# sohmandal/classpose

Hardware: AMD Instinct MI355X
Metric: wsi_tiles_per_sec (higher is better)
Workload: dtype bf16; 1 GPU; configs[1]: synthetic 10000x10000 WSI (1936 tiles), tile 256 / overlap 32, conic 7 classes, ViT-L ClassTransformer depth 24 random-init, batch 32 sub-tiles = 8 WSI tiles/step, every step a distinct batch of the rank's shard (tiles sharded k % n_gpus, at most 256 distinct batches resident, longer runs wrap) streamed pinned host -> hipMemcpyAsync inside the timed region (the reader decodes ahead int; slide=10000, tile=256, overlap=32, batch_subtiles=32, distinct_batches=142, records_gathered=2048, decode_ahead_batches_at_t0=4, device_resident_batches_at_t0=1

## Files before the change

classpose_amd/_lib.py:

```python
from __future__ import annotations

import ctypes as C
import os
import subprocess

_HERE = os.path.dirname(os.path.abspath(__file__))
LIB_PATH = os.path.join(_HERE, "libclasspose_hip.so")
DEBUG_LIB_PATH = os.path.join(_HERE, "libclasspose_hip_debug.so")
CSRC = os.path.join(_HERE, "csrc")

ABI_VERSION = 3
DT_BF16, DT_F16, DT_F32 = 0, 1, 2
DTYPE_CODE = {"bf16": DT_BF16, "fp16": DT_F16, "fp32": DT_F32}
PROF_KINDS = ("fc1", "attention", "qkv", "proj", "fc2", "patch_embed", "neck_head")
FC1_KERNEL_NAME = "k_gemm4w<GELU + folded LayerNorm, one wave per SIMD> = void k_gemm4w<1, 0, false>(Gemm4wArgs)"


class CpxTiling(C.Structure):
    _fields_ = [("H", C.c_int), ("W", C.c_int), ("ypad1", C.c_int), ("xpad1", C.c_int),
                ("Ly", C.c_int), ("Lx", C.c_int), ("ny", C.c_int), ("nx", C.c_int),
                ("bsize", C.c_int), ("augment", C.c_int),
                ("ystart", C.c_int * 16), ("xstart", C.c_int * 16)]


class CpxBlockWeights(C.Structure):
    _fields_ = [(n, C.c_void_p) for n in (
        "ln1_w", "ln1_b", "qkv_w", "qkv_b", "proj_w", "proj_b", "rel_h", "rel_w",
        "ln2_w", "ln2_b", "fc1_w", "fc1_b", "fc2_w", "fc2_b", "qkv_colsum", "fc1_colsum")]


class CpxConvOp(C.Structure):
    _fields_ = [("kind", C.c_int), ("src_a", C.c_int), ("src_b", C.c_int), ("dst", C.c_int),
                ("cin_a", C.c_int), ("cin_b", C.c_int), ("cout", C.c_int), ("h", C.c_int), ("w", C.c_int),
                ("relu", C.c_int), ("weight", C.c_void_p), ("bias", C.c_void_p)]


class CpxQcOp(C.Structure):
    _fields_ = [("kind", C.c_int), ("k", C.c_int), ("stride", C.c_int), ("pad", C.c_int), ("act", C.c_int),
                ("h_in", C.c_int), ("w_in", C.c_int), ("h_out", C.c_int), ("w_out", C.c_int),
                ("src_a", C.c_size_t), ("src_b", C.c_size_t), ("gate", C.c_size_t), ("res", C.c_size_t),
                ("dst", C.c_size_t),
                ("c_a", C.c_int), ("ld_a", C.c_int), ("up_a", C.c_int), ("c_b", C.c_int), ("ld_b", C.c_int),
                ("ld_res", C.c_int), ("c_out", C.c_int), ("ld_dst", C.c_int), ("c_red", C.c_int),
                ("w", C.c_void_p), ("bias", C.c_void_p), ("w2", C.c_void_p), ("bias2", C.c_void_p)]


class CpxNetWeights(C.Structure):
    _fields_ = [("depth", C.c_int), ("ncls", C.c_int), ("n_head_cols", C.c_int),
                ("ld_head", C.c_int), ("dtype", C.c_int), ("fuse_ln", C.c_int),
                ("pe_w", C.c_void_p), ("pe_b", C.c_void_p), ("pos", C.c_void_p),
                ("blocks", C.POINTER(CpxBlockWeights)),
                ("neck0_w", C.c_void_p), ("neck_ln1_w", C.c_void_p), ("neck_ln1_b", C.c_void_p),
                ("neck2_w", C.c_void_p), ("neck_ln2_w", C.c_void_p), ("neck_ln2_b", C.c_void_p),
                ("head_w", C.c_void_p), ("head_b", C.c_void_p),
                ("n_unet_ops", C.c_int), ("unet_ops", C.POINTER(CpxConvOp)), ("prof", C.c_void_p)]


class CpxWeightJob(C.Structure):
    _fields_ = [("op", C.c_int), ("dtype", C.c_int), ("n", C.c_longlong), ("K", C.c_int), ("reserved", C.c_int),
                ("src_host", C.c_void_p * 4), ("stage_off", C.c_size_t * 4), ("dst", C.c_void_p * 3)]


WJ_ROUND_HALF, WJ_ROUND_F32, WJ_COPY_F32, WJ_FOLD_LN = 0, 1, 2, 3


class CpxRecord(C.Structure):
    _fields_ = [("tile", C.c_int32), ("label", C.c_int32), ("cls", C.c_int32), ("area", C.c_int32),
                ("y0", C.c_int32), ("x0", C.c_int32), ("y1", C.c_int32), ("x1", C.c_int32),
                ("sum_y", C.c_int64), ("sum_x", C.c_int64)]


class CpxPqPair(C.Structure):
    _fields_ = [(n, C.c_int32) for n in ("image", "cls", "first_true", "first_pred", "inter", "area_true", "area_pred", "reserved")]


class CpxPqInst(C.Structure):
    _fields_ = [(n, C.c_int32) for n in ("image", "side", "cls", "first", "area", "reserved")]


class CpxCell(C.Structure):
    _fields_ = [("area", C.c_double), ("perimeter", C.c_double), ("cx", C.c_double), ("cy", C.c_double),
                ("n_pts", C.c_int32), ("offset", C.c_int32), ("valid", C.c_int32), ("cls", C.c_int32)]


_p, _i, _f, _d, _sz = C.c_void_p, C.c_int, C.c_float, C.c_double, C.c_size_t

SIGNATURES = {
    "cpx_abi_version": (_i, []),
    "cpx_last_error": (C.c_char_p, []),
    "cpx_build_id": (C.c_char_p, []),
    "cpx_normalize_stats_u8": (_i, [_p, _i, _i, _i, _i, _f, _i, _f, _p, _p, _p]),
    "cpx_normalize_apply_u8": (_i, [_p, _p, _i, _i, _i, _p, _p]),
    "cpx_resize_linear_u8": (_i, [_p, _i, _i, _i, _p, _i, _i, _p]),
    "cpx_make_subtiles": (_i, [_p, _p, _i, C.POINTER(CpxTiling), _p, _p]),
    "cpx_make_patches": (_i, [_p, _p, _i, C.POINTER(CpxTiling), _i, _p, _p]),
    "cpx_make_subtiles_f32": (_i, [_p, _p, _i, C.POINTER(CpxTiling), _p, _p]),
    "cpx_blend_subtiles": (_i, [_p, _i, _i, _i, C.POINTER(CpxTiling), _p, _p, _p, _p, _p]),
    "cpx_blend_subtiles_nchw": (_i, [_p, _p, _i, _i, C.POINTER(CpxTiling), _p, _p, _p, _p, _p]),
    "cpx_qc_forward": (_i, [C.POINTER(CpxQcOp), _i, _p, _i, _i, _i, _sz, _sz, _i, _i, _p, _p, _p, _sz, _p]),
    "cpx_round_weights": (_i, [_p, _p, C.c_longlong, _i, _i, _p]),
    "cpx_fold_layernorm": (_i, [_p, _p, _p, _p, _i, _i, _i, _p, _p, _p, _p]),
    "cpx_weights_build": (_i, [C.POINTER(CpxWeightJob), _i, _p, _sz, _p]),
    "cpx_net_workspace_bytes": (_sz, [_i, _i]),
    "cpx_net_forward": (_i, [C.POINTER(CpxNetWeights), _p, _i, _p, _p, _sz, _p]),
    "cpx_unet_workspace_bytes": (_sz, [C.POINTER(CpxConvOp), _i, _i, _i]),
    "cpx_unet_head_forward": (_i, [C.POINTER(CpxConvOp), _i, _p, _i, _p, _i, _i, _i, _p, _sz, _p]),
    "cpx_net_mlp_parts": (_i, [_i, _i]),
    "cpx_prof_create": (_i, [_i, _i, C.c_uint, C.POINTER(C.c_void_p)]),
    "cpx_prof_collect": (_i, [_p, C.POINTER(C.c_double), C.POINTER(C.c_int)]),
    "cpx_prof_collect_launches": (_i, [_p, C.POINTER(C.c_float), C.POINTER(C.c_int), _i, C.POINTER(C.c_int)]),
    "cpx_prof_destroy": (None, [_p]),
    "cpx_gemm": (_i, [_i, _p, _p, _i, _i, _i, _i, _p, _p, _p, _i, _p]),
    "cpx_gemm_uses_big_tile": (_i, [_i, _i, _i, _i]),
    "cpx_layernorm": (_i, [_i, _p, _p, _p, _i, _i, _f, _p, _p]),
    "cpx_attention": (_i, [_i, _p, _p, _p, _i, _p, _p, _p]),
    "cpx_gemm_bf16": (_i, [_p, _p, _i, _i, _i, _i, _p, _p, _p, _i, _p]),
    "cpx_conv3x3": (_i, [_i, _p, _p, _i, _i, _i, _i, _p, _p, _i, _p]),
    "cpx_gemm_ln": (_i, [_p, _p, _i, _i, _i, _i, _p, _p, _p, _i, _p, _p, _p, _p]),
    "cpx_row_stats": (_i, [_p, _i, _p, _p]),
    "cpx_layernorm_bf16": (_i, [_p, _p, _p, _i, _i, _f, _p, _p]),
    "cpx_attention_relpos": (_i, [_p, _p, _p, _i, _p, _p, _p]),
    "cpx_postproc_workspace_bytes": (_sz, [_i, _i, _i]),
    "cpx_postproc_max_labels": (_i, [_i, _i]),
    "cpx_postproc_launch_count": (C.c_ulonglong, []),
    "cpx_follow_flows": (_i, [_p, _p, _i, _i, _i, _f, _i, _p, _p, _p, _p]),
    "cpx_get_masks": (_i, [_p, _i, _i, _i, _d, _p, _p, _p, _p]),
    "cpx_remove_bad_flow_masks": (_i, [_p, _p, _i, _i, _i, _d, _p, _p, _p]),
    "cpx_fill_holes_and_remove_small_masks": (_i, [_p, _i, _i, _i, _i, _p, _p, _p]),
    "cpx_compute_class_masks": (_i, [_p, _p, _i, _i, _i, _i, _p, _p, _p]),
    "cpx_remove_border_instances": (_i, [_p, _p, _i, _i, _i, _p, _p]),
    "cpx_compute_masks": (_i, [_p, _p, _p, _i, _i, _i, _i, _f, _d, _i, _i, _d, _p, _p, _p, _p, _p]),
    "cpx_instance_records": (_i, [_p, _p, _i, _i, _i, _i, _p, _p, _p, _p]),
    "cpx_compute_masks_records": (_i, [_p, _p, _p, _i, _i, _i, _i, _f, _d, _i, _i, _d, _p, _p, _p, _i, _p, _p, _p, _p]),
    "cpx_resize_linear_f32": (_i, [_p, _i, _i, _i, _p, _i, _i, _p]),
    "cpx_resize_nearest": (_i, [_p, _i, _i, _i, _i, _p, _i, _i, _p]),
    "cpx_pq_workspace_bytes": (_sz, [_i, _i, _i, _i, _i]),
    "cpx_pq_stats": (_i, [_p, _p, _i, _p, _p, _i, _i, _i, _i, _d, _i, _i, _i, _p, _p, _p, _p, _p, _p, _p, _i, _p, _i, _p, _p, _sz, _p]),
    "cpx_net_neck_offset": (_sz, [_i, _i]),
    "cpx_patchify_f32": (_i, [_p, _i, _i, _i, _i, _p, _p]),
    "cpx_class_loss_workspace_bytes": (_sz, [_i, _i, _i, _i]),
    "cpx_class_loss": (_i, [_p, _i, _i, _p, _i, _i, _i, _i, _p, _f, _f, _f, _f, _f, _p, _p, _p, _p, _p, _p, _p, _p, _p, _sz, _p]),
    "cpx_head_wgrad_slab_rows": (_i, []),
    "cpx_head_wgrad_workspace_bytes": (_sz, [_i, _i]),
    "cpx_head_wgrad": (_i, [_p, _p, _i, _i, _i, _p, _p, _p, _sz, _p]),
    "cpx_adamw_step": (_i, [_p, _p, _p, _p, C.c_longlong, _d, _d, _d, _d, _d, _d, _d, _p]),
    "cpx_unet_wgrad_slab_rows": (_i, []),
    "cpx_unet_param_layout": (C.c_longlong, [C.POINTER(CpxConvOp), _i, C.POINTER(C.c_longlong), C.POINTER(C.c_longlong),
                                             C.POINTER(_i), C.POINTER(_i)]),
    "cpx_unet_refresh_operands": (_i, [C.POINTER(CpxConvOp), _i, _p, _i, _p]),
    "cpx_unet_backward_workspace_bytes": (_sz, [C.POINTER(CpxConvOp), _i, _i, _i]),
    "cpx_unet_grad_layout": (_i, [C.POINTER(CpxConvOp), _i, _i, _i, C.POINTER(_sz), C.POINTER(_i)]),
    "cpx_unet_head_backward": (_i, [C.POINTER(CpxConvOp), _i, _p, _i, _i, _p, _sz, _p, _p, _p, _sz, _p]),
    "cpx_net_backbone_offset": (_sz, [_i, _i]),
    "cpx_neck_train_workspace_bytes": (_sz, [_i, _i]),
    "cpx_neck_train_layout": (_i, [_i, _i, C.POINTER(_sz)]),
    "cpx_neck_forward_train": (_i, [C.POINTER(CpxNetWeights), _p, _i, _p, _p, _sz, _p]),
    "cpx_layernorm_backward_workspace_bytes": (_sz, [_i, _i]),
    "cpx_layernorm_backward": (_i, [_i, _p, _p, _p, _i, _i, _f, _p, _p, _p, _p, _sz, _p]),
    "cpx_blocks_train_workspace_bytes": (_sz, [_i, _i, _i]),
    "cpx_blocks_train_layout": (_i, [_i, _i, _i, C.POINTER(_sz)]),
    "cpx_blocks_forward_train": (_i, [C.POINTER(CpxNetWeights), _p, _i, _i, _p, _p, _sz, _p]),
    "cpx_block_grad_layout": (C.c_longlong, [C.POINTER(C.c_longlong)]),
    "cpx_blocks_backward_workspace_bytes": (_sz, [_i, _i]),
    "cpx_blocks_backward_slab_crops": (_i, []),
    "cpx_blocks_backward": (_i, [C.POINTER(CpxNetWeights), _p, _i, _i, _p, _sz, _p, _p, _p, _p, _sz, _p]),
    "cpx_blocks_backward_workspace_bytes_ex": (_sz, [_i, _i, _i]),
    "cpx_blocks_backward_ex": (_i, [C.POINTER(CpxNetWeights), _p, _i, _i, _p, _sz, _p, _i, _p, _p, _p, _sz, _p]),
    "cpx_gemm_tn_bf16": (_i, [_p, _p, _i, _i, _i, _i, _p, _i, _p]),
    "cpx_colsum_workspace_bytes": (_sz, [_i, _i]),
    "cpx_colsum_add": (_i, [_p, _i, _i, _p, _p, _sz, _p]),
    "cpx_layernorm_backward_bytes": (_sz, [_i, _i]),
    "cpx_attention_backward_workspace_bytes": (_sz, [_i]),
    "cpx_attention_backward": (_i, [_i, _p, _p, _p, _p, _p, _i, _p, _p, _p, _p, _sz, _p]),
    "cpx_attention_backward_bf16_workspace_bytes": (_sz, [_i]),
    "cpx_attention_backward_bf16": (_i, [_p, _p, _p, _p, _i, _p, _p, _p, _p, _sz, _p]),
    "cpx_blocks_backward_workspace_bytes_mp": (_sz, [_i, _i, _i, _i]),
    "cpx_blocks_backward_mp": (_i, [C.POINTER(CpxNetWeights), _p, _i, _i, _p, _sz, _p, _i, _i, _p, _p, _p, _sz, _p]),
    "cpx_blocks_backward_in": (_i, [C.POINTER(CpxNetWeights), _p, _i, _i, _p, _sz, _p, _i, _i, _p, _p, _p, _p, _sz, _p]),
    "cpx_gather_crops": (_i, [_i, _p, _i, C.POINTER(_i), _i, _p, _p, _p]),
    "cpx_scatter_crops": (_i, [_i, _p, _i, C.POINTER(_i), _i, _p, _p]),
    "cpx_blocks_train_workspace_bytes_drop": (_sz, [_i, _i, _i]),
    "cpx_blocks_forward_train_drop": (_i, [C.POINTER(CpxNetWeights), _p, _i, _i, _p, _p, _p, _sz, _p]),
    "cpx_blocks_backward_drop": (_i, [C.POINTER(CpxNetWeights), _p, _i, _i, _p, _p, _sz, _p, _i, _i, _p, _p, _p, _p, _sz, _p]),
    "cpx_embed_grad_layout": (C.c_longlong, [C.POINTER(C.c_longlong)]),
    "cpx_embed_backward_workspace_bytes": (_sz, [_i, _i, _i]),
    "cpx_embed_backward": (_i, [_i, _p, _p, _i, _i, _p, _p, _sz, _p]),
    "cpx_gelu_backward": (_i, [_p, _p, _sz, _p, _p]),
    "cpx_neck_grad_layout": (C.c_longlong, [C.POINTER(C.c_longlong)]),
    "cpx_neck_backward_workspace_bytes": (_sz, [_i, _i, _i, C.POINTER(_sz)]),
    "cpx_neck_backward": (_i, [C.POINTER(CpxNetWeights), _p, _i, _p, _sz, _p, _p, _p, _sz, _p]),
    "cpx_hed_jitter_u8": (_i, [_p, _i, _i, _i, _p, _p, _d, _d, _i, _p, _p, _p]),
    "cpx_warp_affine_u8": (_i, [_p, _p, _i, _i, _i, _p, _i, _i, _i, _p, _p, _p]),
    "cpx_warp_affine_f32": (_i, [_p, _p, _i, _i, _i, _p, _i, _i, _i, _p, _p, _p]),
    "cpx_normalize_stats_f32": (_i, [_p, _i, _i, _i, _i, _f, _i, _f, _p, _p]),
    "cpx_normalize_apply_f32": (_i, [_p, _p, _i, _i, _i, _p, _p]),
    "cpx_label_stats_workspace_bytes": (_sz, [_i, _i, _i, _i]),
    "cpx_label_stats": (_i, [_p, _p, _i, _i, _i, _i, _p, _p, _p, _p, _p, _p, _sz, _p]),
    "cpx_rasterize_workspace_bytes": (_sz, [C.c_longlong, C.c_longlong, _i, _i, _i]),
    "cpx_rasterize_polygons": (_i, [_p, _p, _p, _p, C.c_longlong, _i, _i, _i, _p, _p, _sz, _p]),
    "cpx_ids_to_classes": (_i, [_p, C.c_longlong, _p, _i, _p, _p]),
    "cpx_label_components_workspace_bytes": (_sz, [_i, _i, _i]),
    "cpx_label_components": (_i, [_p, _i, _i, _i, _i, _p, _p, _p, _sz, _p]),
    "cpx_distance_sq": (_i, [_p, _i, _i, _i, _p, _p, _sz, _p]),
    "cpx_split_workspace_bytes": (_sz, [_i, _i, _i, _i]),
    "cpx_split_touching": (_i, [_p, _i, _i, _i, _i, _i, _i, _i, _p, _p, _p, _p, _p, _p, _sz, _p]),
    "cpx_pool_byte_sums": (_i, [_p, _p, _p, _i, C.c_longlong, _p, _p, _p]),
    "cpx_warp_affine_pool_u8": (_i, [_p, _p, _p, _p, _i, C.c_longlong, _p, _p, _i, _p, _p, _p, _i, _i, _i, _i, _p, _p, _p, _p]),
    "cpx_stain_samples_workspace_bytes": (_sz, [_i, C.c_longlong]),
    "cpx_stain_samples": (_i, [_p, _p, _p, _i, C.c_longlong, _p, _d, _p, C.c_longlong, _p, _p, _p, _p, _sz, _p]),
    "cpx_he_stain_u8": (_i, [_p, _i, _i, _i, _p, _p, _p, _p, _p]),
    "cpx_warp_affine_pool_stain_u8": (_i, [_p, _p, _p, _p, _i, C.c_longlong, _p, _p, _i, _p, _p, _i, _p, _p, _p, _i, _i, _i, _p, _p,
                                           _p, _p]),
    "cpx_hbs_u8": (_i, [_p, _i, _i, _i, _p, _p, _p, _p, _p]),
    "cpx_blur_pool_rects_u8": (_i, [_p, _p, _p, _i, C.c_longlong, _p, _p, _p, _p, _p, _i, _i, _i, _p, _p, _i, _p, _p, _p, _p,
                                    C.c_longlong, _p, _p]),
    "cpx_warp_affine_pool_quality_u8": (_i, [_p, _p, _p, _p, _i, C.c_longlong, _p, _p, _i, _p, _p, _i, _p, _p, _p, _p, _p, _p, _p,
                                             C.c_longlong, _p, _p, _i, _i, _i, _p, _p, _p, _p]),
    "cpx_masks_to_flows": (_i, [_p, _i, _i, _i, _p, _p, _p, _p]),
    "cpx_warp_affine_pool_flow_f32": (_i, [_p, _p, _p, _i, C.c_longlong, _p, _p, _p, _i, _i, _i, _p, _p, _p]),
    "cpx_seg_loss_workspace_bytes": (_sz, [_i, _i, _i]),
    "cpx_seg_loss": (_i, [_p, _i, _p, _i, _i, _i, _f, _p, _p, _p, _p, _sz, _p]),
    "cpx_find_contours_ccomp_host": (_i, [_p, _i, _i, _p, _i, _p, _p, _p, _i]),
    "cpx_polygonize_workspace_bytes": (_sz, [_i, _i, _i, _i]),
    "cpx_polygonize_device": (_i, [_p, _p, _p, _i, _i, _i, _i, _d, _p, _p, _i, _p, _p, _p, _p]),
    "cpx_polygonize_host": (_i, [_p, _i, _i, _p, _i, _d, _d, _d, _p, _i, _p]),
    "cpx_dedup_pairs_workspace_bytes": (_sz, [_i, _i, _i]),
    "cpx_dedup_pairs": (_i, [_p, _i, _d, _d, _d, _i, _i, _d, _p, C.c_longlong, _p, _p, _sz, _p]),
    "cpx_write_geojson": (_i, [C.c_char_p, C.c_char_p, _p, C.c_int64, _p, _p, _p, _p, C.c_int64, _p, _i, _d, _d, _i]),
    "cpx_write_geojson_ex": (_i, [C.c_char_p, C.c_char_p, _p, C.c_int64, _p, _p, _p, _p, C.c_int64, _p, _i, _d, _d, _i, _p, _i, _p]),
    "cpx_instance_confidence_workspace_bytes": (_sz, [_i, _i, _i, _i, _i]),
    "cpx_instance_confidence": (_i, [_p, _p, _p, _p, _i, _i, _i, _i, _i, _p, _p, _p, _p, _sz, _p]),
}
_PRIVATE = {
    "cpx_gemm_set_variant": (None, [_i]),
    "cpx_attention_set_variant": (None, [_i]),
    "cpx_gemm_set_nt": (None, [_i]),
    "cpx_follow_set_early_exit": (None, [_i]),
    "cpx_blur_set_tile": (None, [_i]),
    "cpx_follow_set_lds_window": (None, [_i]),
    "cpx_gemm_set_reverse": (None, [_i]),
    "cpx_attention_set_xcd_order": (None, [_i]),
    "cpx_gemm_set_big": (None, [_i]),
    "cpx_gemm_set_persistent": (None, [_i]),
    "cpx_gemm_set_persistent_qkv": (None, [_i]),
    "cpx_postproc_set_fused": (None, [_i]),
    "cpx_gemm_set_direct": (None, [_i]),
    "cpx_gemm4w": (_i, [_p, _p, _i, _i, _i, _p, _p, _i, _p]),
    "cpx_gemm4w_set_variant": (None, [_i]),
    "cpx_gemm_set_4w": (None, [_i]),
    "cpx_net_set_mlp_parts": (None, [_i]),
    "cpx_gemm_set_balanced": (None, [_i]),
    "cpx_gemm_set_l2_block": (None, [_i]),
    "cpx_gemm_ln_dt": (_i, [_i, _p, _p, _i, _i, _i, _i, _p, _p, _p, _i, _p, _p, _p, _p]),
    "cpx_row_stats_dt": (_i, [_i, _p, _i, _p, _p]),
    "cpx_im2col3_f32_debug": (_i, [_p, _i, _p, _p]),
    "cpx_confidence_set_footprint": (None, [_i]),
    "cpx_unet_head_layout": (_i, [C.POINTER(CpxConvOp), _i, _i, _i, C.POINTER(_sz), C.POINTER(_i)]),
# ... 109 lines not shown
```

classpose_amd/csrc/cpx_gemm.hip:

```cpp
#include "cpx_internal.h"
#include <type_traits>

typedef __attribute__((ext_vector_type(8))) __bf16 bf16x8;
typedef __attribute__((ext_vector_type(8))) _Float16 f16x8;
typedef __attribute__((ext_vector_type(4))) float f32x4;

#define BM 128
#define BN 128
#define BK 64
#define GEMM_THREADS 256
#define TILE_BYTES (128 * 128)
#define STAGE_BYTES (2 * TILE_BYTES)

template <bool NT_POSSIBLE, bool WT_POSSIBLE = false>
__device__ __forceinline__ void st16(void *p, uint4 v, bool nt, bool wt = false) {
    if (WT_POSSIBLE && wt) {
        typedef unsigned u32x4_t __attribute__((ext_vector_type(4)));
        u32x4_t w = {v.x, v.y, v.z, v.w};
        if (NT_POSSIBLE && nt) asm volatile("global_store_dwordx4 %0, %1, off sc1 nt" ::"v"(p), "v"(w) : "memory");
        else asm volatile("global_store_dwordx4 %0, %1, off sc1" ::"v"(p), "v"(w) : "memory");
    } else if (NT_POSSIBLE && nt) {
        typedef unsigned u32x4_t __attribute__((ext_vector_type(4)));
        u32x4_t w = {v.x, v.y, v.z, v.w};
        __builtin_nontemporal_store(w, reinterpret_cast<u32x4_t *>(p));
    } else {
        *reinterpret_cast<uint4 *>(p) = v;
    }
}
struct GemmArgs {
    const unsigned short *A;
    const unsigned short *W;
    int M, N, K;
    const float *bias;
    const void *aux;
    void *out;
    int ld_out;
    int tiles_n, n_blocks;
    int l2_block;
    int rev_m;
    int nt_out;
    const float *ln_stats;
    const float *ln_colsum;
    float *stats_out;
    int conv_c;
};
#define LN_SLOTS 4
__device__ __forceinline__ float2 ln_mean_rstd(float4 a, float4 b, float inv_k) {
    const float sum = (a.x + a.z) + (b.x + b.z), sq = (a.y + a.w) + (b.y + b.w);
    const float mean = sum * inv_k;
    return make_float2(mean, rsqrtf(fmaxf(sq * inv_k - mean * mean, 0.f) + 1e-6f));
}
__device__ __forceinline__ void ln_row_params(const float *st, int m, float inv_k, float &mean, float &rstd) {
    const float4 a = *reinterpret_cast<const float4 *>(st + (size_t)m * 8);
    const float4 b = *reinterpret_cast<const float4 *>(st + (size_t)m * 8 + 4);
    const float2 p = ln_mean_rstd(a, b, inv_k);
    mean = p.x; rstd = p.y;
}
__device__ __forceinline__ float2 ln_row_scale(float4 a, float4 b, float inv_k) {
    const float2 p = ln_mean_rstd(a, b, inv_k);
    return make_float2(p.y, -p.x * p.y);
}

template <int CTRL, int ROW_MASK = 0xF>
__device__ __forceinline__ float dpp_add(float v) {
    return v + __int_as_float(__builtin_amdgcn_update_dpp(0, __float_as_int(v), CTRL, ROW_MASK, 0xF, false));
}
__device__ __forceinline__ float half_wave_sum(float v) {
    v = dpp_add<0xB1>(v);
    v = dpp_add<0x4E>(v);
    v = dpp_add<0x141>(v);
    v = dpp_add<0x140>(v);
    return dpp_add<0x142, 0xA>(v);
}

template <bool F16>
__device__ __forceinline__ f32x4 mfma16(const uint4 &a, const uint4 &b, f32x4 c) {
    if constexpr (F16)
        return __builtin_amdgcn_mfma_f32_16x16x32_f16(*reinterpret_cast<const f16x8 *>(&a),
                                                      *reinterpret_cast<const f16x8 *>(&b), c, 0, 0, 0);
    else
        return __builtin_amdgcn_mfma_f32_16x16x32_bf16(*reinterpret_cast<const bf16x8 *>(&a),
                                                       *reinterpret_cast<const bf16x8 *>(&b), c, 0, 0, 0);
}

__device__ __forceinline__ float gelu_erf(float x) {
    const float ax = fabsf(x);
    float p = -4.732933965e-04f;
    p = __fmaf_rn(p, ax, 7.084452800e-03f);
    p = __fmaf_rn(p, ax, -5.182713611e-02f);
    p = __fmaf_rn(p, ax, -4.599926953e-01f);
    p = __fmaf_rn(p, ax, -1.150787739e+00f);
    p = __fmaf_rn(p, ax, -1.000037638e+00f);
    const float q = __builtin_amdgcn_exp2f(p);
    return __fmaf_rn(-ax, q, fmaxf(x, 0.0f));
}

template <bool F16>
__device__ __forceinline__ unsigned short to_half(float f) {
    if constexpr (F16) { _Float16 h = (_Float16)f; return *reinterpret_cast<unsigned short *>(&h); }
    else return f32_to_bf16(f);
}
template <bool F16>
__device__ __forceinline__ unsigned pack2(float a, float b) {
    typedef __attribute__((ext_vector_type(2))) float f32x2_t;
    typedef __attribute__((ext_vector_type(2))) __bf16 bf16x2_t;
    typedef __attribute__((ext_vector_type(2))) _Float16 f16x2_t;
    const f32x2_t v = {a, b};
    if constexpr (F16) return __builtin_bit_cast(unsigned, __builtin_convertvector(v, f16x2_t));
    else return __builtin_bit_cast(unsigned, __builtin_convertvector(v, bf16x2_t));
}
template <bool F16>
__device__ __forceinline__ float from_half(unsigned short u) {
    if constexpr (F16) { return (float)*reinterpret_cast<_Float16 *>(&u); }
    else return bf16_to_f32(u);
}

__device__ uint4 g_zero_chunk;

template <bool GLDS, bool CONV = false>
__device__ __forceinline__ void stage_tile(const unsigned short *__restrict__ g, int ldk, int row0, int k0,
                                           char *lds, int tid, uint4 *regs, int conv_c = 0) {
    int dy = 0, dx = 0, c0 = 0;
    if constexpr (CONV) {
        const int tap = k0 / conv_c;
        c0 = k0 - tap * conv_c;
        dy = tap / 3 - 1; dx = tap - (tap / 3) * 3 - 1;
    }
#pragma unroll
    for (int q = 0; q < 4; ++q) {
        int L = q * GEMM_THREADS + tid;
        int row = L >> 3, pc = L & 7;
        int kc = pc ^ (row & 7);
        const unsigned short *src;
        if constexpr (CONV) {
            const int m = row0 + row, yy = ((m >> 5) & 31) + dy, xx = (m & 31) + dx;
            src = ((unsigned)yy < 32u && (unsigned)xx < 32u)
                      ? g + ((size_t)(m & ~1023) + yy * 32 + xx) * conv_c + c0 + kc * 8
                      : reinterpret_cast<const unsigned short *>(&g_zero_chunk);
        } else {
            src = g + (size_t)(row0 + row) * ldk + k0 + kc * 8;
        }
        if constexpr (GLDS) {
            char *base = lds + (q * GEMM_THREADS + (tid & ~63)) * 16;
            __builtin_amdgcn_global_load_lds((const __attribute__((address_space(1))) void *)src,
                                             (__attribute__((address_space(3))) void *)base, 16, 0, 0);
        } else {
            regs[q] = *reinterpret_cast<const uint4 *>(src);
        }
    }
}
__device__ __forceinline__ void write_tile(char *lds, int tid, const uint4 *regs) {
#pragma unroll
    for (int q = 0; q < 4; ++q) *reinterpret_cast<uint4 *>(lds + (q * GEMM_THREADS + tid) * 16) = regs[q];
}

template <int EPI, bool F16, bool GLDS, bool CONV = false>
__global__ void __launch_bounds__(GEMM_THREADS, 2) k_gemm(GemmArgs g) {
    extern __shared__ __attribute__((aligned(16))) char smem[];
    const int tid = threadIdx.x, lane = tid & 63, wave = tid >> 6;
    const int wm = wave >> 1, wn = wave & 1;
    const int bid = xcd_contiguous_id(blockIdx.x, g.n_blocks);
    const int tile_m = bid / g.tiles_n, tile_n = bid - tile_m * g.tiles_n;
    const int m0 = tile_m * BM, n0 = tile_n * BN;
    const int nk = g.K / BK;

    f32x4 acc[4][4];
#pragma unroll
    for (int i = 0; i < 4; ++i)
#pragma unroll
        for (int j = 0; j < 4; ++j) acc[i][j] = (f32x4){0.f, 0.f, 0.f, 0.f};

    uint4 ra[4], rw[4];
    stage_tile<GLDS, CONV>(g.A, g.K, m0, 0, smem, tid, ra, g.conv_c);
    stage_tile<GLDS>(g.W, g.K, n0, 0, smem + TILE_BYTES, tid, rw);
    if constexpr (!GLDS) { write_tile(smem, tid, ra); write_tile(smem + TILE_BYTES, tid, rw); }
    else asm volatile("s_waitcnt vmcnt(0)" ::: "memory");
    __syncthreads();

    const int fr = lane & 15, fq = lane >> 4;
    int offA[2], offW[2];
#pragma unroll
    for (int ks = 0; ks < 2; ++ks) {
        int pc = (ks * 4 + fq) ^ (fr & 7);
        offA[ks] = (wm * 64 + fr) * 128 + pc * 16;
        offW[ks] = TILE_BYTES + (wn * 64 + fr) * 128 + pc * 16;
    }
    for (int kt = 0; kt < nk; ++kt) {
        char *cur = smem + (kt & 1) * STAGE_BYTES;
        char *nxt = smem + ((kt + 1) & 1) * STAGE_BYTES;
        uint4 fa[2][4], fw[2][4];
#pragma unroll
        for (int ks = 0; ks < 2; ++ks)
#pragma unroll
            for (int i = 0; i < 4; ++i) {
                fa[ks][i] = *reinterpret_cast<const uint4 *>(cur + offA[ks] + i * 16 * 128);
                fw[ks][i] = *reinterpret_cast<const uint4 *>(cur + offW[ks] + i * 16 * 128);
            }
        __builtin_amdgcn_sched_barrier(0);
        if (kt + 1 < nk) {
            stage_tile<GLDS, CONV>(g.A, g.K, m0, (kt + 1) * BK, nxt, tid, ra, g.conv_c);
            stage_tile<GLDS>(g.W, g.K, n0, (kt + 1) * BK, nxt + TILE_BYTES, tid, rw);
        }
        __builtin_amdgcn_sched_barrier(0);
#pragma unroll
        for (int ks = 0; ks < 2; ++ks)
#pragma unroll
            for (int nb = 0; nb < 4; ++nb)
#pragma unroll
                for (int mb = 0; mb < 4; ++mb)
                    acc[nb][mb] = mfma16<F16>(fw[ks][nb], fa[ks][mb], acc[nb][mb]);
        __builtin_amdgcn_sched_barrier(0);
        if (kt + 1 < nk) {
            if constexpr (!GLDS) { write_tile(nxt, tid, ra); write_tile(nxt + TILE_BYTES, tid, rw); }
            else asm volatile("s_waitcnt vmcnt(0)" ::: "memory");
        }
        __syncthreads();
    }

#pragma unroll
    for (int mb = 0; mb < 4; ++mb) {
        const int m = m0 + wm * 64 + mb * 16 + fr;
#pragma unroll
        for (int nb = 0; nb < 4; ++nb) {
            const int n = n0 + wn * 64 + nb * 16 + fq * 4;
            f32x4 v = acc[nb][mb];
            if (g.ln_stats) {
                float mean, rstd;
                ln_row_params(g.ln_stats, m, 1.0f / g.K, mean, rstd);
                const float4 cs = *reinterpret_cast<const float4 *>(g.ln_colsum + n);
                v[0] = (v[0] - mean * cs.x) * rstd; v[1] = (v[1] - mean * cs.y) * rstd;
                v[2] = (v[2] - mean * cs.z) * rstd; v[3] = (v[3] - mean * cs.w) * rstd;
            }
            if (g.bias) {
                const float4 b = *reinterpret_cast<const float4 *>(g.bias + n);
                v[0] += b.x; v[1] += b.y; v[2] += b.z; v[3] += b.w;
            }
            if constexpr (EPI == CPX_EPI_GELU_BF16) {
#pragma unroll
                for (int r = 0; r < 4; ++r) v[r] = gelu_erf(v[r]);
            } else if constexpr (EPI == CPX_EPI_RELU_BF16) {
#pragma unroll
                for (int r = 0; r < 4; ++r) v[r] = fmaxf(v[r], 0.f);
            } else if constexpr (EPI == CPX_EPI_RESID_BF16) {
#pragma unroll
                for (int r = 0; r < 4; ++r) v[r] = from_half<F16>(to_half<F16>(v[r]));
                const uint2 rr = *reinterpret_cast<const uint2 *>((const unsigned short *)g.aux + (size_t)m * g.ld_out + n);
                v[0] += from_half<F16>(rr.x & 0xFFFF); v[1] += from_half<F16>(rr.x >> 16);
                v[2] += from_half<F16>(rr.y & 0xFFFF); v[3] += from_half<F16>(rr.y >> 16);
            } else if constexpr (EPI == CPX_EPI_POS_BF16) {
                const float4 p = *reinterpret_cast<const float4 *>((const float *)g.aux + (size_t)(m & 1023) * g.N + n);
                v[0] += p.x; v[1] += p.y; v[2] += p.z; v[3] += p.w;
            }
            if constexpr (EPI == CPX_EPI_F32) {
                *reinterpret_cast<float4 *>((float *)g.out + (size_t)m * g.ld_out + n) = make_float4(v[0], v[1], v[2], v[3]);
            } else if (EPI == CPX_EPI_QKV_BF16 && n >= 2048) {
                unsigned short *vT = (unsigned short *)g.aux;
                const size_t s_ = (size_t)(m >> 10), t_ = (size_t)(m & 1023);
#pragma unroll
                for (int r = 0; r < 4; ++r) {
                    const int c = n - 2048 + r;
                    vT[((s_ * 16 + (c >> 6)) * 64 + (c & 63)) * 1024 + t_] = to_half<F16>(v[r]);
                }
            } else {
                uint2 o;
                o.x = pack2<F16>(v[0], v[1]);
                o.y = pack2<F16>(v[2], v[3]);
                *reinterpret_cast<uint2 *>((unsigned short *)g.out + (size_t)m * g.ld_out + n) = o;
            }
        }
    }
}


typedef __attribute__((ext_vector_type(4))) unsigned u32x4;
#define G2_THREADS 512
#define G2_HALF 16384
#define G2_BUF 65536
#define G2_EPI_LD 528
#define G2_LN_OFF (256 * G2_EPI_LD)
#define G2_LDS_BYTES (G2_LN_OFF + 256 * 8)

template <int OFF>
__device__ __forceinline__ u32x4 lds_read128(unsigned addr) {
    u32x4 v;
    asm volatile("ds_read_b128 %0, %1 offset:%2" : "=v"(v) : "v"(addr), "n"(OFF));
    return v;
}
template <bool F16>
__device__ __forceinline__ f32x4 mfma16v(const u32x4 &a, const u32x4 &b, f32x4 c) {
    if constexpr (F16)
        return __builtin_amdgcn_mfma_f32_16x16x32_f16(__builtin_bit_cast(f16x8, a), __builtin_bit_cast(f16x8, b), c, 0, 0, 0);
    else
        return __builtin_amdgcn_mfma_f32_16x16x32_bf16(__builtin_bit_cast(bf16x8, a), __builtin_bit_cast(bf16x8, b), c, 0, 0, 0);
}
template <int HM>
__device__ __forceinline__ void g2_read_x(u32x4 (&fx)[4][2], unsigned b0, unsigned b1) {
    fx[0][0] = lds_read128<HM * G2_HALF + 0 * 2048>(b0); fx[0][1] = lds_read128<HM * G2_HALF + 0 * 2048>(b1);
    fx[1][0] = lds_read128<HM * G2_HALF + 1 * 2048>(b0); fx[1][1] = lds_read128<HM * G2_HALF + 1 * 2048>(b1);
    fx[2][0] = lds_read128<HM * G2_HALF + 2 * 2048>(b0); fx[2][1] = lds_read128<HM * G2_HALF + 2 * 2048>(b1);
    fx[3][0] = lds_read128<HM * G2_HALF + 3 * 2048>(b0); fx[3][1] = lds_read128<HM * G2_HALF + 3 * 2048>(b1);
}
template <int HN>
__device__ __forceinline__ void g2_read_w(u32x4 (&fw)[2][2], unsigned b0, unsigned b1) {
    fw[0][0] = lds_read128<(2 + HN) * G2_HALF + 0 * 2048>(b0); fw[0][1] = lds_read128<(2 + HN) * G2_HALF + 0 * 2048>(b1);
    fw[1][0] = lds_read128<(2 + HN) * G2_HALF + 1 * 2048>(b0); fw[1][1] = lds_read128<(2 + HN) * G2_HALF + 1 * 2048>(b1);
}
template <bool F16, bool FIRST = false>
__device__ __forceinline__ void g2_mma(f32x4 (&acc)[4][2], const u32x4 (&fx)[4][2], const u32x4 (&fw)[2][2]) {
    __builtin_amdgcn_s_setprio(1);
#pragma unroll
    for (int ks = 0; ks < 2; ++ks)
#pragma unroll
        for (int mb = 0; mb < 4; ++mb)
#pragma unroll
            for (int nb = 0; nb < 2; ++nb)
                acc[mb][nb] = mfma16v<F16>(fw[nb][ks], fx[mb][ks], (FIRST && ks == 0) ? (f32x4){0.f, 0.f, 0.f, 0.f} : acc[mb][nb]);
    __builtin_amdgcn_s_setprio(0);
}
#define G2_BAR() __builtin_amdgcn_s_barrier()
#define G2_LGKM0() do { asm volatile("s_waitcnt lgkmcnt(0)" ::: "memory"); __builtin_amdgcn_sched_barrier(0); } while (0)

#define G2_TILE_OF(bid, tiles_m, tile_m, tile_n)                                            \
    if (g.l2_block && ((tiles_m) & 7) == 0 && (g.tiles_n & 3) == 0) {                       \
        const int grp = bid >> 5, w_ = bid & 31, cgn = g.tiles_n >> 2, rgn = (tiles_m) >> 3; \
        const int rg = g.l2_block == 2 ? grp % rgn : grp / cgn, cg = g.l2_block == 2 ? grp / rgn : grp - rg * cgn; \
        tile_m = rg * 8 + (w_ >> 2);                                                        \
        tile_n = cg * 4 + (w_ & 3);                                                         \
    } else {                                                                                \
        tile_m = bid / g.tiles_n;                                                           \
        tile_n = bid - tile_m * g.tiles_n;                                                  \
    }
#define G2_FRAG_BASES(xb, wb)                                                               \
    _Pragma("unroll") for (int ks = 0; ks < 2; ++ks) {                                      \
        const unsigned sw = (unsigned)(((ks * 4 + fq) ^ (fr & 7)) << 4);                    \
        xb[0][ks] = lds0 + (wm * 64 + fr) * 128 + sw;                                       \
        wb[0][ks] = lds0 + (wn * 32 + fr) * 128 + sw;                                       \
        xb[1][ks] = xb[0][ks] + G2_BUF;                                                     \
        wb[1][ks] = wb[0][ks] + G2_BUF;                                                     \
    }
#define G2_PHASES(B, FIRST, C1, C2)                                                         \
                                                                                    \
        g2_read_w<0>(fw, wb[B][0], wb[B][1]);                                               \
        g2_read_x<0>(fx, xb[B][0], xb[B][1]);                                               \
        if (C1) stage(1, t_ + 1);                                                           \
        G2_BAR(); G2_LGKM0();                                                               \
        g2_mma<F16, FIRST>(acc[0][0], fx, fw);                                              \
        __builtin_amdgcn_sched_barrier(0); G2_BAR();                                        \
                                                                                    \
        g2_read_w<1>(fw, wb[B][0], wb[B][1]);                                               \
        if (C1) stage(2, t_ + 1);                                                           \
        G2_BAR(); G2_LGKM0();                                                               \
        g2_mma<F16, FIRST>(acc[0][1], fx, fw);                                              \
        __builtin_amdgcn_sched_barrier(0); G2_BAR();                                        \
                                                                                    \
        g2_read_x<1>(fx, xb[B][0], xb[B][1]);                                               \
        if (C2) stage(0, t_ + 2);                                                           \
        G2_BAR(); G2_LGKM0();                                                               \
        g2_mma<F16, FIRST>(acc[1][1], fx, fw);                                              \
        __builtin_amdgcn_sched_barrier(0); G2_BAR();                                        \
                                                                                    \
        g2_read_w<0>(fw, wb[B][0], wb[B][1]);                                               \
        if (C2) { stage(3, t_ + 2); asm volatile("s_waitcnt vmcnt(4)" ::: "memory"); }      \
        else if (C1) asm volatile("s_waitcnt vmcnt(0)" ::: "memory");                       \
        G2_BAR(); G2_LGKM0();                                                               \
        g2_mma<F16, FIRST>(acc[1][0], fx, fw);                                              \
        __builtin_amdgcn_sched_barrier(0); G2_BAR();
#define G2_EPI_VALUE(v, rs, nm, cs, b)                                                      \
    {                                                                                       \
        if constexpr (LN_IN) {                                                              \
            v[0] = fmaf(v[0], rs, fmaf(nm, (cs).x, (b).x)); v[1] = fmaf(v[1], rs, fmaf(nm, (cs).y, (b).y)); \
            v[2] = fmaf(v[2], rs, fmaf(nm, (cs).z, (b).z)); v[3] = fmaf(v[3], rs, fmaf(nm, (cs).w, (b).w)); \
        } else {                                                                            \
            v[0] += (b).x; v[1] += (b).y; v[2] += (b).z; v[3] += (b).w;                     \
        }                                                                                   \
        if constexpr (EPI == CPX_EPI_GELU_BF16) {                                           \
            _Pragma("unroll") for (int r = 0; r < 4; ++r) v[r] = gelu_erf(v[r]);            \
        } else if constexpr (EPI == CPX_EPI_RELU_BF16) {                                    \
            _Pragma("unroll") for (int r = 0; r < 4; ++r) v[r] = fmaxf(v[r], 0.f);          \
        }                                                                                   \
    }
#define G2_STAGE_VT(v, nl, ml)                                                              \
    {                                                                                       \
        const unsigned p01 = pack2<F16>(v[0], v[1]), p23 = pack2<F16>(v[2], v[3]);          \
        *reinterpret_cast<unsigned short *>(smem + (nl + 0) * G2_EPI_LD + ml * 2) = (unsigned short)p01; \
        *reinterpret_cast<unsigned short *>(smem + (nl + 1) * G2_EPI_LD + ml * 2) = (unsigned short)(p01 >> 16); \
        *reinterpret_cast<unsigned short *>(smem + (nl + 2) * G2_EPI_LD + ml * 2) = (unsigned short)p23; \
        *reinterpret_cast<unsigned short *>(smem + (nl + 3) * G2_EPI_LD + ml * 2) = (unsigned short)(p23 >> 16); \
    }
#define G2_STORE_VT_ROWS(STORE)                                                             \
    {                                                                                       \
        unsigned short *vT = (unsigned short *)g.aux;                                       \
        const size_t s_ = (size_t)(m0 >> 10), t0 = (size_t)(m0 & 1023);                     \
        _Pragma("unroll 4") for (int it = 0; it < 16; ++it) {                               \
            const int row = it * 16 + (tid >> 5);                                           \
            const int c = n0 - 2048 + row;                                                  \
            uint4 v_ = *reinterpret_cast<const uint4 *>(smem + row * G2_EPI_LD + c16 * 16); \
            unsigned short *p_ = vT + ((s_ * 16 + (c >> 6)) * 64 + (c & 63)) * 1024 + t0 + c16 * 8; \
            STORE;                                                                          \
        }                                                                                   \
    }
#define G2_ADD_RESID(v, rres_it)                                                            \
    {                                                                                       \
        const uint4 rr = rres_it;                                                           \
        unsigned a[4] = {v.x, v.y, v.z, v.w}, b[4] = {rr.x, rr.y, rr.z, rr.w};              \
        _Pragma("unroll") for (int i = 0; i < 4; ++i) {                                     \
            float lo = from_half<F16>(a[i] & 0xFFFF) + from_half<F16>(b[i] & 0xFFFF);       \
            float hi = from_half<F16>(a[i] >> 16) + from_half<F16>(b[i] >> 16);             \
// ... 374 lines not shown
            const unsigned ldb = (unsigned)g.ld_out * 2u;
            const unsigned ovoff = (unsigned)(wm * 64 + fr) * ldb + (unsigned)(wn * 32 + ((fq & 1) << 4) + ((fq >> 1) << 3)) * 2u;
            const unsigned so0 = (unsigned)m0 * ldb + (unsigned)n0 * 2u;
#pragma unroll
            for (int hm = 0; hm < 2; ++hm) {
                float ln_rs[4], ln_nm[4];
                if constexpr (LN_IN) {
#pragma unroll
                    for (int mb = 0; mb < 4; ++mb) {
                        const float2 pr = *reinterpret_cast<const float2 *>(smem + G2P_TAIL + (hm * 128 + wm * 64 + mb * 16 + fr) * 8);
                        ln_rs[mb] = pr.x; ln_nm[mb] = pr.y;
                    }
                }
#pragma unroll
                for (int hn = 0; hn < 2; ++hn) {
                    float4 b[2], cs[2];
#pragma unroll
                    for (int nb = 0; nb < 2; ++nb) {
                        const int nl = hn * 128 + wn * 32 + nb * 16 + fq * 4;
                        b[nb] = *reinterpret_cast<const float4 *>(smem + G2P_TAIL + 2048 + nl * 4);
                        cs[nb] = make_float4(0.f, 0.f, 0.f, 0.f);
                        if constexpr (LN_IN) cs[nb] = *reinterpret_cast<const float4 *>(smem + G2P_TAIL + 3072 + nl * 4);
                    }
#pragma unroll
                    for (int mb = 0; mb < 4; ++mb) {
                        unsigned pk[2][2];
#pragma unroll
                        for (int nb = 0; nb < 2; ++nb) {
                            f32x4 vv = acc[hm][hn][mb][nb];
                            G2_EPI_VALUE(vv, ln_rs[mb], ln_nm[mb], cs[nb], b[nb])
                            pk[nb][0] = pack2<F16>(vv[0], vv[1]);
                            pk[nb][1] = pack2<F16>(vv[2], vv[3]);
                        }
                        const auto r0 = __builtin_amdgcn_permlane16_swap(pk[0][0], pk[1][0], false, false);
                        const auto r1 = __builtin_amdgcn_permlane16_swap(pk[0][1], pk[1][1], false, false);
                        const u32x4 o = {r0[0], r1[0], r0[1], r1[1]};
                        __builtin_amdgcn_raw_buffer_store_b128(o, rsrcO, ovoff, so0 + (unsigned)(hm * 128 + mb * 16) * ldb + (unsigned)hn * 256u, 0);
                    }
                }
            }
            G2_BAR();
        } else {
            if constexpr (EPI != CPX_EPI_RESID_BF16) {
                if (has_next) prefetch_next();
            }
            char *stg = smem + G2P_STG_OFF;
#pragma unroll
            for (int hm = 0; hm < 2; ++hm) {
                uint4 rres[8];
                if constexpr (EPI == CPX_EPI_RESID_BF16) {
#pragma unroll
                    for (int it = 0; it < 8; ++it)
                        rres[it] = *reinterpret_cast<const uint4 *>((const unsigned short *)g.aux +
                                                                    (size_t)(m0 + hm * 128 + it * 16 + (tid >> 5)) * g.ld_out + n0 + c16 * 8);
                }
                float ln_rs[4], ln_nm[4];
                if constexpr (LN_IN) {
#pragma unroll
                    for (int mb = 0; mb < 4; ++mb) {
                        const float2 pr = *reinterpret_cast<const float2 *>(smem + G2P_TAIL + (hm * 128 + wm * 64 + mb * 16 + fr) * 8);
                        ln_rs[mb] = pr.x; ln_nm[mb] = pr.y;
                    }
                }
#pragma unroll
                for (int hn = 0; hn < 2; ++hn)
#pragma unroll
                    for (int nb = 0; nb < 2; ++nb) {
                        const int nl = hn * 128 + wn * 32 + nb * 16 + fq * 4;
                        const float4 b = *reinterpret_cast<const float4 *>(smem + G2P_TAIL + 2048 + nl * 4);
                        float4 cs = make_float4(0.f, 0.f, 0.f, 0.f);
                        if constexpr (LN_IN) cs = *reinterpret_cast<const float4 *>(smem + G2P_TAIL + 3072 + nl * 4);
#pragma unroll
                        for (int mb = 0; mb < 4; ++mb) {
                            const int mlh = wm * 64 + mb * 16 + fr;
                            f32x4 vv = acc[hm][hn][mb][nb];
                            G2_EPI_VALUE(vv, ln_rs[mb], ln_nm[mb], cs, b)
                            uint2 o;
                            o.x = pack2<F16>(vv[0], vv[1]);
                            o.y = pack2<F16>(vv[2], vv[3]);
                            *reinterpret_cast<uint2 *>(stg + mlh * G2_EPI_LD + nl * 2) = o;
                        }
                    }
                asm volatile("s_waitcnt lgkmcnt(0)" ::: "memory");
                G2_BAR();
#pragma unroll
                for (int it = 0; it < 8; ++it) {
                    const int mlh = it * 16 + (tid >> 5);
                    uint4 vv = *reinterpret_cast<const uint4 *>(stg + mlh * G2_EPI_LD + c16 * 16);
                    const int ml = hm * 128 + mlh;
                    const size_t go = (size_t)(m0 + ml) * g.ld_out + n0 + c16 * 8;
                    if constexpr (EPI == CPX_EPI_RESID_BF16) G2_ADD_RESID(vv, rres[it])
                    st16<EPI == CPX_EPI_QKV_BF16, EPI == CPX_EPI_RESID_BF16 || EPI == CPX_EPI_QKV_BF16>((unsigned short *)g.out + go, vv, (g.nt_out & (n0 < 1024 ? 1 : 2)) != 0,
                                                                                        (g.nt_out & (EPI == CPX_EPI_QKV_BF16 ? 16 : 8)) != 0);
                    if constexpr (STATS) g2_row_stats<F16>(vv, c16, g.stats_out, (size_t)(m0 + ml), tile_n);
                }
                asm volatile("s_waitcnt lgkmcnt(0)" ::: "memory");
                G2_BAR();
            }
        }
        if (!has_next) break;
        prefetched = next_issued;
        v = vn; m0 = m0n; n0 = n0n; tile_n = tile_nn;
    }
}
#undef G2_TILE_OF
#undef G2_FRAG_BASES
#undef G2_PHASES
#undef G2_EPI_VALUE
#undef G2_STAGE_VT
#undef G2_STORE_VT_ROWS
#undef G2_ADD_RESID

CPX_SWITCH(g_gemm_persist, 1);
CPX_SWITCH(g_gemm_variant, 1);
CPX_SWITCH(g_gemm_l2, 1);
CPX_SWITCH(g_gemm_persist_qkv, 1);
CPX_SWITCH(g_gemm_rev, 0);
CPX_SWITCH(g_gemm_big, 1);
CPX_SWITCH(g_gemm_bal, 1);
CPX_SWITCH(g_gemm_direct, 1);
CPX_SWITCH(g_gemm_nt, 15);
CPX_SWITCH(g_gemm_4w, 1);
#ifdef CPX_DEBUG
extern "C" void cpx_gemm_set_persistent(int on) { g_gemm_persist = on; }
extern "C" void cpx_gemm_set_variant(int glds) { g_gemm_variant = glds; }
extern "C" void cpx_gemm_set_persistent_qkv(int on) { g_gemm_persist_qkv = on; }
extern "C" void cpx_gemm_set_l2_block(int on) { g_gemm_l2 = on; }
extern "C" void cpx_gemm_set_reverse(int on) { g_gemm_rev = on; }
extern "C" void cpx_gemm_set_big(int on) { g_gemm_big = on; }
extern "C" void cpx_gemm_set_direct(int on) { g_gemm_direct = on; }
extern "C" void cpx_gemm_set_balanced(int on) { g_gemm_bal = on; }
extern "C" void cpx_gemm_set_4w(int on) { g_gemm_4w = on; }
extern "C" void cpx_gemm_set_nt(int on) { g_gemm_nt = on; }
#endif

#define CPX_F16_DISPATCH(f16, F16, ...)                               \
    do {                                                              \
        if (f16) { constexpr bool F16 = true; __VA_ARGS__; }          \
        else { constexpr bool F16 = false; __VA_ARGS__; }             \
    } while (0)
template <auto KERNEL, int LDS_BYTES>
static void gemm_allow_lds() {
    static CpxOncePerDevice once;
    once([] { (void)hipFuncSetAttribute((const void *)KERNEL, hipFuncAttributeMaxDynamicSharedMemorySize, LDS_BYTES); });
}
static int gemm_cu_count() {
    int dev = 0, cus = 256;
    (void)hipGetDevice(&dev);
    (void)hipDeviceGetAttribute(&cus, hipDeviceAttributeMultiprocessorCount, dev);
    return cus > 0 ? cus : 256;
}

int cpx_gemm_half_uses_big_tile(int M, int N, int K, int epilogue) {
    if (epilogue == CPX_EPI_F32) return 0;
    if (!g_gemm_big || M % 256 || N % 256 || K < 128) return 0;
    if ((K / 64) % 2 && epilogue != CPX_EPI_POS_BF16) return 0;
    return (M / 256) * (N / 256) >= 256;
}

template <int EPI, bool F16, int FLAGS>
static void launch_gemm256_tiles(const GemmArgs &a, hipStream_t s) {
    gemm_allow_lds<k_gemm256<EPI, F16, FLAGS>, G2_LDS_BYTES>();
    hipLaunchKernelGGL((k_gemm256<EPI, F16, FLAGS>), dim3(a.n_blocks), dim3(G2_THREADS), G2_LDS_BYTES, s, a);
}
template <int EPI, bool F16, int FLAGS>
static void launch_gemm256_flags(const GemmArgs &a, hipStream_t s) {
    const bool qkv_balanced = EPI == CPX_EPI_QKV_BF16 && g_gemm_persist_qkv && (a.n_blocks / a.tiles_n) % 64 == 0 && a.tiles_n == 12;
    const bool fits32 = (size_t)a.M * (size_t)a.K * 2 < ((size_t)1 << 31) && (size_t)a.N * (size_t)a.K * 2 < ((size_t)1 << 31);
    if (g_gemm_persist && fits32 && (EPI != CPX_EPI_QKV_BF16 || qkv_balanced)) {
        gemm_allow_lds<k_gemm256p<EPI, F16, FLAGS>, G2P_LDS_BYTES>();
        static const int n_cu = gemm_cu_count();
        if (EPI == CPX_EPI_QKV_BF16) {
            if (n_cu == 256) {
                GemmArgs b = a;
                b.l2_block = 3;
                hipLaunchKernelGGL((k_gemm256p<EPI, F16, FLAGS>), dim3(256), dim3(G2_THREADS), G2P_LDS_BYTES, s, b);
                return;
            }
        } else {
            const int grid = a.n_blocks < n_cu ? a.n_blocks : n_cu;
            hipLaunchKernelGGL((k_gemm256p<EPI, F16, FLAGS>), dim3(grid), dim3(G2_THREADS), G2P_LDS_BYTES, s, a);
            return;
        }
    }
    launch_gemm256_tiles<EPI, F16, FLAGS>(a, s);
}

template <int EPI, bool F16>
static bool launch_gemm256(const GemmArgs &a0, hipStream_t s) {
    if constexpr (EPI == CPX_EPI_F32) return false;
    else {
        if (!cpx_gemm_half_uses_big_tile(a0.M, a0.N, a0.K, EPI)) return false;
        GemmArgs a = a0;
        a.tiles_n = a.N / 256; a.n_blocks = (a.M / 256) * (a.N / 256);
        constexpr bool PRODUCER = EPI == CPX_EPI_RESID_BF16 || EPI == CPX_EPI_POS_BF16;
        constexpr int F1 = PRODUCER ? G2F_STATS : G2F_LN;
        const bool f1 = PRODUCER ? a.stats_out != nullptr : a.ln_stats != nullptr;
        if constexpr (EPI == CPX_EPI_POS_BF16) {
            if (!f1) launch_gemm256_tiles<EPI, F16, 0>(a, s);
            else launch_gemm256_tiles<EPI, F16, G2F_STATS>(a, s);
            return true;
        } else {
            if constexpr (EPI == CPX_EPI_GELU_BF16) {
                if (g_gemm_4w && f1 && a.bias && a.K >= 256 && (a.K / 64) % 2 == 0 &&
                    cpx_gemm4w_gelu_ln(F16 ? 1 : 0, a.A, a.W, a.M, a.N, a.K, a.bias, a.ln_stats, a.ln_colsum, a.out, a.ld_out, s))
                    return true;
            }
            constexpr bool DIRECT_OK = EPI == CPX_EPI_GELU_BF16
#ifdef CPX_DEBUG
                                       || (EPI != CPX_EPI_RESID_BF16 && EPI != CPX_EPI_QKV_BF16)
#endif
                ;
            constexpr bool BAL_OK = EPI == CPX_EPI_RESID_BF16 && !F16;
            const bool bal = BAL_OK && g_gemm_bal != 0 && f1 && a.K >= 256;
            if constexpr (DIRECT_OK) {
                if ((EPI == CPX_EPI_GELU_BF16 ? g_gemm_direct != 0 : g_gemm_direct == 2) && (size_t)a.M * (size_t)a.ld_out * 2 < ((size_t)1 << 31)) {
                    if (f1) launch_gemm256_flags<EPI, F16, F1 | G2F_DIRECT>(a, s);
                    else launch_gemm256_flags<EPI, F16, G2F_DIRECT>(a, s);
                    return true;
                }
            }
            if constexpr (BAL_OK) {
                if (bal) {
                    launch_gemm256_flags<EPI, F16, F1 | G2F_BAL>(a, s);
                    return true;
                }
            }
            if (f1) launch_gemm256_flags<EPI, F16, F1>(a, s);
            else launch_gemm256_flags<EPI, F16, 0>(a, s);
            return true;
        }
    }
}

template <int EPI>
static void launch_gemm(const GemmArgs &a, hipStream_t s, bool f16) {
    bool big;
    CPX_F16_DISPATCH(f16, F16, big = launch_gemm256<EPI, F16>(a, s));
    if (big) return;
    dim3 grid(a.n_blocks), block(GEMM_THREADS);
    size_t lds = 2 * STAGE_BYTES;
#ifdef CPX_DEBUG
    if (!g_gemm_variant) {
        CPX_F16_DISPATCH(f16, F16, hipLaunchKernelGGL((k_gemm<EPI, F16, false>), grid, block, lds, s, a));
        return;
    }
#endif
    CPX_F16_DISPATCH(f16, F16, hipLaunchKernelGGL((k_gemm<EPI, F16, true>), grid, block, lds, s, a));
}

template <bool F16>
__device__ __forceinline__ void row_stats_emit(const uint4 a, const uint4 b, int lane, size_t row, float *__restrict__ st) {
    const unsigned u[8] = {a.x, a.y, a.z, a.w, b.x, b.y, b.z, b.w};
    float sm = 0.f, sq = 0.f;
#pragma unroll
    for (int i = 0; i < 8; ++i) {
        const float lo = from_half<F16>(u[i] & 0xFFFF), hi = from_half<F16>(u[i] >> 16);
        sm += lo + hi; sq += lo * lo + hi * hi;
    }
#pragma unroll
    for (int o = 32; o > 0; o >>= 1) { sm += __shfl_xor(sm, o); sq += __shfl_xor(sq, o); }
    if (lane < 4) *reinterpret_cast<float2 *>(st + (row * LN_SLOTS + lane) * 2) = lane == 0 ? make_float2(sm, sq) : make_float2(0.f, 0.f);
}
template <bool F16>
__global__ void __launch_bounds__(256) k_row_stats(const unsigned short *__restrict__ x, int rows,
                                                   float *__restrict__ st) {
    const int lane = threadIdx.x & 63, row = blockIdx.x * 4 + (threadIdx.x >> 6);
    if (row >= rows) return;
    const unsigned short *xr = x + (size_t)row * 1024 + lane * 16;
    const uint4 a = *reinterpret_cast<const uint4 *>(xr), b = *reinterpret_cast<const uint4 *>(xr + 8);
    row_stats_emit<F16>(a, b, lane, (size_t)row, st);
}

template <int NV, int STATS>
__global__ void __launch_bounds__(256) k_move_crop_rows(const uint4 *__restrict__ src, uint4 *__restrict__ dst, CpxCropList list, int scatter,
                                                        float *__restrict__ st) {
    const int lane = threadIdx.x & 63, tok = blockIdx.x * 4 + (threadIdx.x >> 6);
    const size_t crow = (size_t)(list.first + blockIdx.y) * 1024 + tok, frow = (size_t)list.crop[blockIdx.y] * 1024 + tok;
    const uint4 *s = src + (scatter ? crow : frow) * (64 * NV) + lane * NV;
    uint4 *d = dst + (scatter ? frow : crow) * (64 * NV) + lane * NV;
    uint4 v[NV];
#pragma unroll
    for (int i = 0; i < NV; ++i) v[i] = s[i];
#pragma unroll
    for (int i = 0; i < NV; ++i) d[i] = v[i];
    if constexpr (STATS != 0) row_stats_emit<STATS == 2>(v[0], v[1], lane, crow, st);
}
int cpx_move_crop_rows_run(int dtype, const void *src, void *dst, const CpxCropList &list, int scatter, float *stats, hipStream_t s) {
    const dim3 grid(256, list.n), block(256);
    const uint4 *a = (const uint4 *)src;
    uint4 *b = (uint4 *)dst;
    if (dtype == CPX_DT_F32) hipLaunchKernelGGL((k_move_crop_rows<4, 0>), grid, block, 0, s, a, b, list, scatter, stats);
    else if (!stats || scatter) hipLaunchKernelGGL((k_move_crop_rows<2, 0>), grid, block, 0, s, a, b, list, scatter, stats);
    else if (dtype == CPX_DT_F16) hipLaunchKernelGGL((k_move_crop_rows<2, 2>), grid, block, 0, s, a, b, list, scatter, stats);
    else hipLaunchKernelGGL((k_move_crop_rows<2, 1>), grid, block, 0, s, a, b, list, scatter, stats);
    CPX_CHECK_LAUNCH();
    return CPX_OK;
}
int cpx_row_stats_half(int dtype, const void *x, int rows, float *stats, void *stream) {
    CPX_REQUIRE(x && stats && rows > 0 && (dtype == CPX_DT_BF16 || dtype == CPX_DT_F16));
    CPX_F16_DISPATCH(dtype == CPX_DT_F16, F16,
                     hipLaunchKernelGGL(k_row_stats<F16>, dim3(cpx_cdiv(rows, 4)), dim3(256), 0, (hipStream_t)stream, (const unsigned short *)x, rows, stats));
    CPX_CHECK_LAUNCH();
    return CPX_OK;
}

extern "C" int cpx_row_stats(const void *x, int rows, float *stats, void *stream) {
    return cpx_row_stats_half(CPX_DT_BF16, x, rows, stats, stream);
}

static GemmArgs gemm_args(const void *A, const void *Wt, int M, int N, int K, const float *bias, const void *aux, void *out, int ld_out) {
    GemmArgs a = {};
    a.A = (const unsigned short *)A; a.W = (const unsigned short *)Wt;
    a.M = M; a.N = N; a.K = K; a.bias = bias; a.aux = aux; a.out = out; a.ld_out = ld_out;
    a.tiles_n = N / BN; a.n_blocks = (M / BM) * (N / BN);
    return a;
}

int cpx_gemm_half(int dtype, const void *A, const void *Wt, int M, int N, int K, int epilogue,
                  const float *bias, const void *aux, void *out, int ld_out,
                  const float *ln_stats, const float *ln_colsum, float *stats_out, void *stream) {
    CPX_REQUIRE(A && Wt && out && (dtype == CPX_DT_BF16 || dtype == CPX_DT_F16));
    const bool f16 = dtype == CPX_DT_F16;
    CPX_REQUIRE(M > 0 && N > 0 && K > 0 && M % BM == 0 && N % BN == 0 && K % BK == 0);
    CPX_REQUIRE(ld_out >= N && ld_out % 4 == 0);
    CPX_REQUIRE((epilogue != CPX_EPI_RESID_BF16 && epilogue != CPX_EPI_POS_BF16 && epilogue != CPX_EPI_QKV_BF16) || aux);
    CPX_REQUIRE(epilogue != CPX_EPI_QKV_BF16 || (N == 3072 && M % 1024 == 0));
    CPX_REQUIRE(!ln_stats || (ln_colsum && epilogue != CPX_EPI_RESID_BF16));
    CPX_REQUIRE(!stats_out || ((epilogue == CPX_EPI_RESID_BF16 || epilogue == CPX_EPI_POS_BF16) && N == 1024 && cpx_gemm_half_uses_big_tile(M, N, K, epilogue)));
    GemmArgs a = gemm_args(A, Wt, M, N, K, bias, aux, out, ld_out);
    a.ln_stats = ln_stats; a.ln_colsum = ln_colsum; a.stats_out = stats_out; a.l2_block = g_gemm_l2; a.nt_out = g_gemm_nt;
    a.rev_m = (g_gemm_rev && K >= 4096) ? 1 : 0;
    hipStream_t s = (hipStream_t)stream;
    switch (epilogue) {
        case CPX_EPI_BF16: launch_gemm<CPX_EPI_BF16>(a, s, f16); break;
        case CPX_EPI_GELU_BF16: launch_gemm<CPX_EPI_GELU_BF16>(a, s, f16); break;
        case CPX_EPI_RESID_BF16: launch_gemm<CPX_EPI_RESID_BF16>(a, s, f16); break;
        case CPX_EPI_F32: launch_gemm<CPX_EPI_F32>(a, s, f16); break;
        case CPX_EPI_POS_BF16: launch_gemm<CPX_EPI_POS_BF16>(a, s, f16); break;
        case CPX_EPI_RELU_BF16: launch_gemm<CPX_EPI_RELU_BF16>(a, s, f16); break;
        case CPX_EPI_QKV_BF16: launch_gemm<CPX_EPI_QKV_BF16>(a, s, f16); break;
        default: CPX_REQUIRE(!"unknown epilogue");
    }
    CPX_CHECK_LAUNCH();
    return CPX_OK;
}

int cpx_conv3_half(int dtype, const void *x, const void *Wt, int M, int N, int C, int epilogue, const float *bias,
                   void *out, int ld_out, void *stream) {
    CPX_REQUIRE(x && Wt && out && (dtype == CPX_DT_BF16 || dtype == CPX_DT_F16));
    CPX_REQUIRE(M > 0 && M % 1024 == 0 && N > 0 && N % BN == 0 && C > 0 && C % BK == 0);
    CPX_REQUIRE(ld_out >= N && ld_out % 4 == 0 && (epilogue == CPX_EPI_BF16 || epilogue == CPX_EPI_RELU_BF16));
    GemmArgs a = gemm_args(x, Wt, M, N, 9 * C, bias, nullptr, out, ld_out);
    a.conv_c = C;
    hipStream_t s = (hipStream_t)stream;
    dim3 grid(a.n_blocks), block(GEMM_THREADS);
    const size_t lds = 2 * STAGE_BYTES;
    const bool f16 = dtype == CPX_DT_F16;
    if (epilogue == CPX_EPI_BF16) CPX_F16_DISPATCH(f16, F16, hipLaunchKernelGGL((k_gemm<CPX_EPI_BF16, F16, true, true>), grid, block, lds, s, a));
    else CPX_F16_DISPATCH(f16, F16, hipLaunchKernelGGL((k_gemm<CPX_EPI_RELU_BF16, F16, true, true>), grid, block, lds, s, a));
    CPX_CHECK_LAUNCH();
    return CPX_OK;
}

extern "C" int cpx_conv3x3(int dtype, const void *x, const void *Wt, int M, int N, int C, int epilogue, const float *bias,
                           void *out, int ld_out, void *stream) {
    return cpx_conv3_half(dtype, x, Wt, M, N, C, epilogue, bias, out, ld_out, stream);
}

extern "C" int cpx_gemm_ln(const void *A, const void *Wt, int M, int N, int K, int epilogue,
                           const float *bias, const void *aux, void *out, int ld_out,
                           const float *ln_stats, const float *ln_colsum, float *stats_out, void *stream) {
    return cpx_gemm_half(CPX_DT_BF16, A, Wt, M, N, K, epilogue, bias, aux, out, ld_out, ln_stats, ln_colsum, stats_out, stream);
}
#ifdef CPX_DEBUG
extern "C" int cpx_gemm_ln_dt(int dtype, const void *A, const void *Wt, int M, int N, int K, int epilogue,
                              const float *bias, const void *aux, void *out, int ld_out,
                              const float *ln_stats, const float *ln_colsum, float *stats_out, void *stream) {
    return cpx_gemm_half(dtype, A, Wt, M, N, K, epilogue, bias, aux, out, ld_out, ln_stats, ln_colsum, stats_out, stream);
}
#endif
#ifdef CPX_DEBUG
extern "C" int cpx_row_stats_dt(int dtype, const void *x, int rows, float *stats, void *stream) {
    return cpx_row_stats_half(dtype, x, rows, stats, stream);
}
#endif
extern "C" int cpx_gemm_bf16(const void *A, const void *Wt, int M, int N, int K, int epilogue,
                             const float *bias, const void *aux, void *out, int ld_out, void *stream) {
    return cpx_gemm_half(CPX_DT_BF16, A, Wt, M, N, K, epilogue, bias, aux, out, ld_out, nullptr, nullptr, nullptr, stream);
}
extern "C" int cpx_gemm(int dtype, const void *A, const void *Wt, int M, int N, int K, int epilogue,
                        const float *bias, const void *aux, void *out, int ld_out, void *stream) {
    if (dtype == CPX_DT_F32)
        return cpx_gemm_f32((const float *)A, (const float *)Wt, M, N, K, epilogue, bias, (const float *)aux, (float *)out, ld_out, stream);
    return cpx_gemm_half(dtype, A, Wt, M, N, K, epilogue, bias, aux, out, ld_out, nullptr, nullptr, nullptr, stream);
}
extern "C" int cpx_gemm_uses_big_tile(int M, int N, int K, int epilogue) { return cpx_gemm_half_uses_big_tile(M, N, K, epilogue); }
```

classpose_amd/csrc/cpx_internal.h:

```cpp
#pragma once
#include "cpx_common.h"
#include <atomic>

struct CpxOncePerDevice {
    std::atomic<unsigned long long> done{0};
    template <class F>
    void operator()(F &&f) {
        int dev = 0;
        (void)hipGetDevice(&dev);
        const unsigned long long bit = 1ull << (dev & 63);
        if (!(done.load(std::memory_order_acquire) & bit)) {
            f();
            done.fetch_or(bit, std::memory_order_release);
        }
    }
};

enum { CPX_PROF_FC1 = 0, CPX_PROF_ATTN = 1, CPX_PROF_QKV = 2, CPX_PROF_PROJ = 3, CPX_PROF_FC2 = 4,
       CPX_PROF_PE = 5,
       CPX_PROF_TAIL = 6,
       CPX_PROF_KINDS = 7 };
struct CpxProf {
    hipEvent_t *ev = nullptr;
    int *kind = nullptr;
    int cap = 0, n = 0, stride = 1;
    int phase = 0;
    unsigned kinds_mask = 1;
};
static inline bool cpx_prof_begin(CpxProf *p, int kind, int layer, hipStream_t s) {
    if (!p || !p->ev || p->n >= p->cap || !((p->kinds_mask >> kind) & 1)) return false;
    if (kind < CPX_PROF_PE && ((layer + p->phase) % p->stride) != 0) return false;
    p->kind[p->n] = kind;
    return hipEventRecord(p->ev[2 * p->n], s) == hipSuccess;
}
static inline void cpx_prof_end(CpxProf *p, hipStream_t s) {
    (void)hipEventRecord(p->ev[2 * p->n + 1], s);
    ++p->n;
}

int cpx_gemm_half(int dtype, const void *A, const void *Wt, int M, int N, int K, int epilogue, const float *bias,
                  const void *aux, void *out, int ld_out, const float *ln_stats, const float *ln_colsum,
                  float *stats_out, void *stream);
int cpx_conv3_half(int dtype, const void *x, const void *Wt, int M, int N, int C, int epilogue, const float *bias,
                   void *out, int ld_out, void *stream);
int cpx_row_stats_half(int dtype, const void *x, int rows, float *stats, void *stream);
int cpx_gemm_half_uses_big_tile(int M, int N, int K, int epilogue);
#define CPX_CROP_LIST 64
struct CpxCropList { int n, first; int crop[CPX_CROP_LIST]; };
int cpx_move_crop_rows_run(int dtype, const void *src, void *dst, const CpxCropList &list, int scatter, float *stats, hipStream_t s);
int cpx_gemm4w_gelu_ln(int f16, const void *A, const void *W, int M, int N, int K, const float *bias, const float *ln_stats, const float *ln_colsum,
                       void *out, int ld_out, hipStream_t s);
int cpx_layernorm_half(int dtype, const void *x, const float *w, const float *b, int rows, int C, float eps,
                       void *out, void *stream);
int cpx_attention_half(int dtype, const void *qkv, const void *rel_h, const void *rel_w, int n_subtiles, void *vT_ws,
                       void *out, void *stream, bool transpose_v);
int cpx_attention2w_launch(int dtype, const void *qkv, const void *vT, const void *rel_h, const void *rel_w,
                           int n_subtiles, void *out, int xcd_order, hipStream_t s);

int cpx_gemm_f32(const float *A, const float *Wt, int M, int N, int K, int epilogue, const float *bias,
                 const float *aux, float *out, int ld_out, void *stream);
int cpx_layernorm_f32(const float *x, const float *w, const float *b, int rows, int C, float eps, float *out,
                      void *stream);
int cpx_attention_f32(const float *qkv, const float *rel_h, const float *rel_w, int n_subtiles, float *out,
                      void *stream);
int cpx_im2col3_f32(const float *x, int n_subtiles, float *out, void *stream);

__device__ __forceinline__ int xcd_contiguous_id(int v, int nblk) {
    const int nxcd = 8, q = nblk / nxcd, r = nblk % nxcd, x = v % nxcd;
    return (x < r ? x * (q + 1) : r * (q + 1) + (x - r) * q) + v / nxcd;
}

#define CPX_RUN(call) do { const int rc_ = (call); if (rc_) return rc_; } while (0)

struct NetWs { size_t off_x, off_xn, off_qkv, off_vt, off_ao, off_h, off_neck, off_neck2, off_st, off_col, total; };
NetWs cpx_net_ws(int nS, int dtype);
struct CpxBlockBufs { const void *x_in; void *x_mid, *x_out, *xn, *qkv, *vt, *ao, *hb; float *st; };
int cpx_net_block(const cpx_net_weights *w, int layer, int nS, const CpxBlockBufs &t, bool big_stats, CpxProf *prof, void *stream);
bool cpx_net_big_stats(const cpx_net_weights *w, int nS);
int cpx_net_tail(const cpx_net_weights *w, const void *x, int nS, void *y0, void *a1, void *y2, void *feat, void *col, float *head,
                 void *unet_ws, size_t unet_ws_bytes, void *stream);

int cpx_unet_head_run(int dtype, const cpx_conv_op *ops, int n_ops, const void *feat, int nS, float *head, int ld_head,
                      int col0, void *workspace, size_t ws_bytes, void *stream);
size_t cpx_unet_ws_bytes(int dtype, const cpx_conv_op *ops, int n_ops, int nS);
void cpx_unet_act_layout(int dtype, const cpx_conv_op *ops, int n_ops, int nS, size_t *off, int *ld);

static inline size_t es_of(int dtype) { return dtype == CPX_DT_F32 ? 4 : 2; }
static inline bool dtype_ok(int dtype) { return dtype == CPX_DT_BF16 || dtype == CPX_DT_F16 || dtype == CPX_DT_F32; }
static inline int up128(long long x) { return (int)((x + 127) / 128 * 128); }
static inline int up64(int x) { return (x + 63) / 64 * 64; }
struct OpDims { int taps, ctot, Npad, Kpad, Kp128, ho, wo, ld, rows_pad, rows_out_pad; size_t rows; };
static inline OpDims op_dims(const cpx_conv_op &o, int nS) {
    OpDims d;
    d.taps = o.kind == 0 ? 9 : (o.kind == 1 ? 4 : 1);
    d.ctot = o.cin_a + o.cin_b;
    d.Npad = up128(o.kind == 2 ? 4 * o.cout : o.cout);
    d.Kpad = up64(d.taps * d.ctot);
    d.Kp128 = up128(d.Kpad);
    d.ho = o.kind == 0 ? o.h : (o.kind == 1 ? o.h / 2 : o.h * 2);
    d.wo = o.kind == 0 ? o.w : (o.kind == 1 ? o.w / 2 : o.w * 2);
    d.rows = o.kind == 2 ? (size_t)nS * o.h * o.w : (size_t)nS * d.ho * d.wo;
    d.ld = up128(o.cout);
    d.rows_pad = up128((long long)d.rows);
    d.rows_out_pad = up128((long long)nS * d.ho * d.wo);
    return d;
}
struct CpxTensor { const char *p; int ld, c, h, w; };

#define CPX_DT_DISPATCH(dtype, DT, ...)                                                   \
    do {                                                                                  \
        if ((dtype) == CPX_DT_BF16) { constexpr int DT = CPX_DT_BF16; __VA_ARGS__; }      \
        else if ((dtype) == CPX_DT_F16) { constexpr int DT = CPX_DT_F16; __VA_ARGS__; }   \
        else { constexpr int DT = CPX_DT_F32; __VA_ARGS__; }                              \
    } while (0)
template <int DT>
__device__ __forceinline__ float load_f32(const void *p, size_t idx) {
    if constexpr (DT == CPX_DT_F32) return ((const float *)p)[idx];
    else if constexpr (DT == CPX_DT_F16) return (float)((const _Float16 *)p)[idx];
    else return bf16_to_f32(((const unsigned short *)p)[idx]);
}
template <int DT>
__device__ __forceinline__ float half_bits_to_f32(unsigned u) {
    if constexpr (DT == CPX_DT_F16) { const unsigned short h = (unsigned short)u; return (float)*reinterpret_cast<const _Float16 *>(&h); }
    else return bf16_to_f32((unsigned short)u);
}
template <int DT>
__device__ __forceinline__ float4 ld4(const void *p, size_t idx) {
    if constexpr (DT == CPX_DT_F32) return *reinterpret_cast<const float4 *>((const float *)p + idx);
    else {
        const uint2 a = *reinterpret_cast<const uint2 *>((const unsigned short *)p + idx);
        return make_float4(half_bits_to_f32<DT>(a.x & 0xFFFF), half_bits_to_f32<DT>(a.x >> 16), half_bits_to_f32<DT>(a.y & 0xFFFF),
                           half_bits_to_f32<DT>(a.y >> 16));
    }
}
typedef __attribute__((ext_vector_type(16))) float f32x16;
#define MFMA_F32(a, b, c) __builtin_amdgcn_mfma_f32_32x32x2f32((a), (b), (c), 0, 0, 0)
static inline dim3 grid1(size_t n) { return dim3((unsigned)((n + 255) / 256)); }
__device__ __forceinline__ double wave_sum(double x) {
#pragma unroll
    for (int o = 32; o > 0; o >>= 1) x += __shfl_xor(x, o, 64);
    return x;
}

struct AttnBwdLayout { size_t off_st[3], off_b[4], off_part, total; };
static inline AttnBwdLayout cpx_attn_bwd_layout(int nS) {
    AttnBwdLayout L; CpxArena a; const size_t n = (size_t)nS * 16 * 1024;
    for (int i = 0; i < 3; ++i) L.off_st[i] = a.take(n * sizeof(float));
    for (int i = 0; i < 4; ++i) L.off_b[i] = a.take(n * 32 * sizeof(float));
    L.off_part = a.take((size_t)nS * 4 * 2 * 4096 * sizeof(double));
    L.total = a.o;
    return L;
}
int cpx_attn_rel_grad_run(int dtype, const void *qkv, const float *Gh, const float *Gw, double *part, int nS, int add_rel, float *drel_h,
                          float *drel_w, void *stream);
int cpx_attention_backward_bf16_run(const void *qkv, const void *rel_h, const void *rel_w, const float *dO, int nS, float *dqkv, float *drel_h,
                                    float *drel_w, int add_rel, void *workspace, size_t workspace_bytes, void *stream);

#define UW_SLAB 512

struct UwArgs {
    const float *dy;
    const void *xa, *xb;
    int lda, ca, ldb, cb;
    int lh, lw;
    int rows, Npad, Kpad, k_valid;
    float *part_w; double *part_b;
};
struct DxArgs {
    const float *dcol; int ldc;
    int kind, ctot, coff, C;
    int lh, lw;
    size_t rows_src;
    float *gx; int ld_gx;
    const void *y; int ld_y; int mask;
};
size_t cpx_uwgrad_part_w_bytes(size_t rows, int Npad, int Kpad);
size_t cpx_uwgrad_workspace_bytes(size_t rows, int Npad, int Kpad);
int cpx_uwgrad_run(int dtype, int kind, const UwArgs &u, int n_valid, int bias_taps, int cout, float *dW, float *db, hipStream_t s);
int cpx_wt_run(int dtype, const void *w, int Npad, int Kpad, int Kp128, float *wt, hipStream_t s);
int cpx_dx_gather_run(int dtype, const DxArgs &g, hipStream_t s);
int cpx_transpose_f32_run(int dtype, const void *in, int R, int Cc, float *out, hipStream_t s);
```

classpose_amd/csrc/cpx_net.hip:

```cpp
#include "cpx_internal.h"
#include <algorithm>

typedef __attribute__((ext_vector_type(8))) __bf16 bf16x8;
typedef __attribute__((ext_vector_type(8))) _Float16 f16x8;

template <bool F16>
__device__ __forceinline__ f32x16 mfma32(const uint4 &a, const uint4 &b, f32x16 c) {
    if constexpr (F16)
        return __builtin_amdgcn_mfma_f32_32x32x16_f16(*reinterpret_cast<const f16x8 *>(&a),
                                                      *reinterpret_cast<const f16x8 *>(&b), c, 0, 0, 0);
    else
        return __builtin_amdgcn_mfma_f32_32x32x16_bf16(*reinterpret_cast<const bf16x8 *>(&a),
                                                       *reinterpret_cast<const bf16x8 *>(&b), c, 0, 0, 0);
}
template <bool F16>
__device__ __forceinline__ unsigned short h_from_f32(float f) {
    if constexpr (F16) { _Float16 h = (_Float16)f; return *reinterpret_cast<unsigned short *>(&h); }
    else return f32_to_bf16(f);
}
template <bool F16>
__device__ __forceinline__ float f32_from_h(unsigned short u) {
    if constexpr (F16) return (float)*reinterpret_cast<_Float16 *>(&u);
    else return bf16_to_f32(u);
}
// ... 291 lines not shown
    unsigned short *orow = out + (tok0 + qh * 32 + r) * 1024 + head * 64;
#pragma unroll
    for (int db = 0; db < 2; ++db)
#pragma unroll
        for (int g4 = 0; g4 < 4; g4 += 2) {
            const f32x16 &O = db ? O1 : O0;
            unsigned ax = pack2<F16>(O[4 * g4 + 0] * inv, O[4 * g4 + 1] * inv), ay = pack2<F16>(O[4 * g4 + 2] * inv, O[4 * g4 + 3] * inv);
            unsigned bx = pack2<F16>(O[4 * g4 + 4] * inv, O[4 * g4 + 5] * inv), by = pack2<F16>(O[4 * g4 + 6] * inv, O[4 * g4 + 7] * inv);
            const auto rx = __builtin_amdgcn_permlane32_swap(ax, bx, false, false);
            const auto ry = __builtin_amdgcn_permlane32_swap(ay, by, false, false);
            *reinterpret_cast<uint4 *>(orow + db * 32 + 8 * g4 + 8 * h2) = make_uint4(rx[0], ry[0], rx[1], ry[1]);
        }
}

CPX_SWITCH(g_att_xcd, 1);
CPX_SWITCH(g_att_v8, 2);
#ifdef CPX_DEBUG
extern "C" void cpx_attention_set_variant(int v8) { g_att_v8 = v8; }
extern "C" void cpx_attention_set_xcd_order(int v) { g_att_xcd = v; }
#endif
extern "C" int cpx_attention_relpos(const void *qkv, const void *rel_h, const void *rel_w,
                                    int n_subtiles, void *vT_ws, void *out, void *stream) {
    return cpx_attention_half(CPX_DT_BF16, qkv, rel_h, rel_w, n_subtiles, vT_ws, out, stream, true);
}
extern "C" int cpx_attention(int dtype, const void *qkv, const void *rel_h, const void *rel_w,
                             int n_subtiles, void *vT_ws, void *out, void *stream) {
    if (dtype == CPX_DT_F32)
        return cpx_attention_f32((const float *)qkv, (const float *)rel_h, (const float *)rel_w, n_subtiles, (float *)out, stream);
    return cpx_attention_half(dtype, qkv, rel_h, rel_w, n_subtiles, vT_ws, out, stream, true);
}
int cpx_attention_half(int dtype, const void *qkv, const void *rel_h, const void *rel_w, int n_subtiles,
                       void *vT_ws, void *out, void *stream, bool transpose_v) {
    CPX_REQUIRE(qkv && rel_h && rel_w && vT_ws && out && n_subtiles > 0);
    CPX_REQUIRE(dtype == CPX_DT_BF16 || dtype == CPX_DT_F16);
#ifdef CPX_DEBUG
    CPX_REQUIRE(g_att_v8 == 2 || g_att_v8 == 7);
#endif
    hipStream_t s = (hipStream_t)stream;
    if (transpose_v)
        hipLaunchKernelGGL(k_v_transpose, dim3(16, 16, n_subtiles), dim3(256), 0, s,
                           (const unsigned short *)qkv, (unsigned short *)vT_ws);
#ifdef CPX_DEBUG
    if (g_att_v8 == 7) {
        const dim3 grid4(8, 16, n_subtiles);
        static CpxOncePerDevice once4;
        once4([] {
            (void)hipFuncSetAttribute((const void *)k_attention4p<true>, hipFuncAttributeMaxDynamicSharedMemorySize, A4_LDS_BYTES);
            (void)hipFuncSetAttribute((const void *)k_attention4p<false>, hipFuncAttributeMaxDynamicSharedMemorySize, A4_LDS_BYTES);
        });
        if (dtype == CPX_DT_F16)
            hipLaunchKernelGGL((k_attention4p<true>), grid4, dim3(ATT_THREADS), A4_LDS_BYTES, s, (const unsigned short *)qkv, (const unsigned short *)vT_ws,
                               (const unsigned short *)rel_h, (const unsigned short *)rel_w, (unsigned short *)out, g_att_xcd);
        else
            hipLaunchKernelGGL((k_attention4p<false>), grid4, dim3(ATT_THREADS), A4_LDS_BYTES, s, (const unsigned short *)qkv, (const unsigned short *)vT_ws,
                               (const unsigned short *)rel_h, (const unsigned short *)rel_w, (unsigned short *)out, g_att_xcd);
        CPX_CHECK_LAUNCH();
        return CPX_OK;
    }
#endif
    return cpx_attention2w_launch(dtype, qkv, vT_ws, rel_h, rel_w, n_subtiles, out, g_att_xcd, s);
}

NetWs cpx_net_ws(int nS, int dtype) {
    NetWs w; CpxArena a; const size_t M = (size_t)nS * 1024, es = es_of(dtype);
    w.off_x = a.take(M * 1024 * es);
    w.off_xn = a.take(M * 1024 * es);
    w.off_qkv = a.take(M * 3072 * es);
    w.off_vt = a.take(es == 2 ? M * 1024 * es : 0);
    w.off_ao = a.take(M * 1024 * es);
    w.off_h = a.take(M * 4096 * es);
    w.off_neck = a.take(M * 256 * es);
    w.off_neck2 = a.take(M * 256 * es);
    w.off_st = a.take(es == 2 ? M * 8 * sizeof(float) : 0);
    w.off_col = a.take(es == 4 ? M * 2304 * es : 0);
    w.total = a.o;
    return w;
}
extern "C" size_t cpx_net_workspace_bytes(int n_subtiles, int dtype) {
    return n_subtiles > 0 ? cpx_net_ws(n_subtiles, dtype).total : 0;
}

extern "C" size_t cpx_net_neck_offset(int n_subtiles, int dtype) {
    if (n_subtiles <= 0 || dtype < CPX_DT_BF16 || dtype > CPX_DT_F32) return 0;
    return cpx_net_ws(n_subtiles, dtype).off_neck2;
}

extern "C" size_t cpx_net_backbone_offset(int n_subtiles, int dtype) {
    if (n_subtiles <= 0 || dtype < CPX_DT_BF16 || dtype > CPX_DT_F32) return (size_t)-1;
    return cpx_net_ws(n_subtiles, dtype).off_x;
}

extern "C" int cpx_prof_create(int max_launches, int stride, unsigned kinds_mask, void **out) {
    CPX_REQUIRE(out && max_launches > 0);
    CpxProf *p = new CpxProf();
    p->ev = new hipEvent_t[2 * (size_t)max_launches];
    p->kind = new int[max_launches];
    for (int i = 0; i < 2 * max_launches; ++i) {
        hipError_t e = hipEventCreate(&p->ev[i]);
        if (e != hipSuccess) {
            for (int j = 0; j < i; ++j) (void)hipEventDestroy(p->ev[j]);
            delete[] p->ev; delete[] p->kind; delete p;
            CPX_HIP(e);
        }
    }
    p->cap = max_launches; p->n = 0; p->stride = stride > 0 ? stride : 1;
    p->kinds_mask = kinds_mask ? kinds_mask : 1u;
    *out = p;
    return CPX_OK;
}
extern "C" int cpx_prof_collect(void *prof, double *ms_sum, int *count) {
    CpxProf *p = (CpxProf *)prof;
    CPX_REQUIRE(p && ms_sum && count);
    for (int k = 0; k < CPX_PROF_KINDS; ++k) { ms_sum[k] = 0.0; count[k] = 0; }
    for (int i = 0; i < p->n; ++i) {
        float ms = 0.f;
        CPX_HIP(hipEventElapsedTime(&ms, p->ev[2 * i], p->ev[2 * i + 1]));
        ms_sum[p->kind[i]] += ms;
        ++count[p->kind[i]];
    }
    p->n = 0;
    return CPX_OK;
}
extern "C" int cpx_prof_collect_launches(void *prof, float *ms, int *kind, int cap, int *n_out) {
    CpxProf *p = (CpxProf *)prof;
    CPX_REQUIRE(p && ms && kind && n_out && cap >= 0);
    for (int i = 0; i < p->n && i < cap; ++i) {
        CPX_HIP(hipEventElapsedTime(&ms[i], p->ev[2 * i], p->ev[2 * i + 1]));
        kind[i] = p->kind[i];
    }
    *n_out = p->n;
    return CPX_OK;
}
extern "C" void cpx_prof_destroy(void *prof) {
    CpxProf *p = (CpxProf *)prof;
    if (!p) return;
    for (int i = 0; i < 2 * p->cap; ++i) (void)hipEventDestroy(p->ev[i]);
    delete[] p->ev; delete[] p->kind; delete p;
}

CPX_SWITCH(g_mlp_parts, 1);
#ifdef CPX_DEBUG
extern "C" void cpx_net_set_mlp_parts(int on) { g_mlp_parts = on; }
#endif
extern "C" int cpx_net_mlp_parts(int n_subtiles, int dtype) {
    if (!g_mlp_parts || dtype == CPX_DT_F32 || n_subtiles < 32) return 1;
    return n_subtiles / 16;
}
static void mlp_part_rows(int n_subtiles, int parts, int pt, int &row0, int &rows) {
    row0 = pt * 16384;
    rows = pt + 1 < parts ? 16384 : n_subtiles * 1024 - row0;
}

int cpx_net_tail(const cpx_net_weights *w, const void *x, int nS, void *y0, void *a1, void *y2, void *feat, void *col, float *head,
                 void *unet_ws, size_t unet_ws_bytes, void *stream) {
    const int dt = w->dtype, M = nS * 1024;
    CPX_RUN(cpx_gemm(dt, x, w->neck0_w, M, 256, 1024, CPX_EPI_BF16, nullptr, nullptr, y0, 256, stream));
    CPX_RUN(cpx_layernorm(dt, y0, w->neck_ln1_w, w->neck_ln1_b, M, 256, 1e-6f, a1, stream));
    if (dt == CPX_DT_F32) {
        CPX_RUN(cpx_im2col3_f32((const float *)a1, nS, (float *)col, stream));
        CPX_RUN(cpx_gemm(dt, col, w->neck2_w, M, 256, 2304, CPX_EPI_BF16, nullptr, nullptr, y2, 256, stream));
    } else {
        CPX_RUN(cpx_conv3_half(dt, a1, w->neck2_w, M, 256, 256, CPX_EPI_BF16, nullptr, y2, 256, stream));
    }
    CPX_RUN(cpx_layernorm(dt, y2, w->neck_ln2_w, w->neck_ln2_b, M, 256, 1e-6f, feat, stream));
    CPX_RUN(cpx_gemm(dt, feat, w->head_w, M, w->ld_head, 256, CPX_EPI_F32, w->head_b, nullptr, head, w->ld_head, stream));
    if (w->n_unet_ops > 0) {
        const size_t need = cpx_unet_ws_bytes(dt, w->unet_ops, w->n_unet_ops, nS);
        CPX_REQUIRE(unet_ws_bytes >= need);
        CPX_RUN(cpx_unet_head_run(dt, w->unet_ops, w->n_unet_ops, feat, nS, head, w->ld_head, 192, unet_ws, need, stream));
    }
    return CPX_OK;
}

#define TIMED(kind_, layer_, call_) do { const bool t_ = cpx_prof_begin(prof, kind_, layer_, hs); CPX_RUN(call_); if (t_) cpx_prof_end(prof, hs); } while (0)

bool cpx_net_big_stats(const cpx_net_weights *w, int nS) {
    const int M = nS * 1024;
    return w->fuse_ln && w->dtype != CPX_DT_F32 && cpx_gemm_half_uses_big_tile(M, 1024, 1024, CPX_EPI_RESID_BF16) &&
           cpx_gemm_half_uses_big_tile(M, 1024, 4096, CPX_EPI_RESID_BF16);
}

int cpx_net_block(const cpx_net_weights *w, int layer, int nS, const CpxBlockBufs &t, bool big_stats, CpxProf *prof, void *stream) {
    const cpx_block_weights &b = w->blocks[layer];
    const int dt = w->dtype, M = nS * 1024;
    const bool f32 = dt == CPX_DT_F32;
    hipStream_t hs = (hipStream_t)stream;
    auto attention = [&] {
        return f32 ? cpx_attention_f32((const float *)t.qkv, (const float *)b.rel_h, (const float *)b.rel_w, nS, (float *)t.ao, stream)
                   : cpx_attention_half(dt, t.qkv, b.rel_h, b.rel_w, nS, t.vt, t.ao, stream, false);
    };
    if (w->fuse_ln) {
        TIMED(CPX_PROF_QKV, layer, cpx_gemm_half(dt, t.x_in, b.qkv_w, M, 3072, 1024, CPX_EPI_QKV_BF16, b.qkv_b, t.vt, t.qkv, 3072, t.st, b.qkv_colsum, nullptr, stream));
        TIMED(CPX_PROF_ATTN, layer, attention());
        TIMED(CPX_PROF_PROJ, layer, cpx_gemm_half(dt, t.ao, b.proj_w, M, 1024, 1024, CPX_EPI_RESID_BF16, b.proj_b, t.x_in, t.x_mid, 1024, nullptr, nullptr, big_stats ? t.st : nullptr, stream));
        if (!big_stats) CPX_RUN(cpx_row_stats_half(dt, t.x_mid, M, t.st, stream));
        const int parts = big_stats ? cpx_net_mlp_parts(nS, dt) : 1;
        for (int pt = 0; pt < parts; ++pt) {
            int r0, Mp;
            mlp_part_rows(nS, parts, pt, r0, Mp);
            const char *xp = (const char *)t.x_mid + (size_t)r0 * 1024 * 2;
            char *op = (char *)t.x_out + (size_t)r0 * 1024 * 2;
            float *stp = t.st + (size_t)r0 * 8;
            TIMED(CPX_PROF_FC1, layer, cpx_gemm_half(dt, xp, b.fc1_w, Mp, 4096, 1024, CPX_EPI_GELU_BF16, b.fc1_b, nullptr, t.hb, 4096, stp, b.fc1_colsum, nullptr, stream));
            TIMED(CPX_PROF_FC2, layer, cpx_gemm_half(dt, t.hb, b.fc2_w, Mp, 1024, 4096, CPX_EPI_RESID_BF16, b.fc2_b, xp, op, 1024, nullptr, nullptr, big_stats ? stp : nullptr, stream));
        }
        if (!big_stats) CPX_RUN(cpx_row_stats_half(dt, t.x_out, M, t.st, stream));
        return CPX_OK;
    }
    CPX_RUN(cpx_layernorm(dt, t.x_in, b.ln1_w, b.ln1_b, M, 1024, 1e-6f, t.xn, stream));
    TIMED(CPX_PROF_QKV, layer, cpx_gemm(dt, t.xn, b.qkv_w, M, 3072, 1024, f32 ? CPX_EPI_F32 : CPX_EPI_QKV_BF16, b.qkv_b, f32 ? nullptr : t.vt, t.qkv, 3072, stream));
    TIMED(CPX_PROF_ATTN, layer, attention());
    TIMED(CPX_PROF_PROJ, layer, cpx_gemm(dt, t.ao, b.proj_w, M, 1024, 1024, CPX_EPI_RESID_BF16, b.proj_b, t.x_in, t.x_mid, 1024, stream));
    CPX_RUN(cpx_layernorm(dt, t.x_mid, b.ln2_w, b.ln2_b, M, 1024, 1e-6f, t.xn, stream));
    TIMED(CPX_PROF_FC1, layer, cpx_gemm(dt, t.xn, b.fc1_w, M, 4096, 1024, CPX_EPI_GELU_BF16, b.fc1_b, nullptr, t.hb, 4096, stream));
    TIMED(CPX_PROF_FC2, layer, cpx_gemm(dt, t.hb, b.fc2_w, M, 1024, 4096, CPX_EPI_RESID_BF16, b.fc2_b, t.x_mid, t.x_out, 1024, stream));
    return CPX_OK;
}

extern "C" int cpx_net_forward(const cpx_net_weights *w, const void *patches, int nS, float *head,
                               void *workspace, size_t workspace_bytes, void *stream) {
    CPX_REQUIRE(w && patches && head && workspace && nS > 0);
    CPX_REQUIRE(w->depth > 0 && w->blocks && w->ld_head % 128 == 0 && w->ld_head >= w->n_head_cols);
    CPX_REQUIRE(dtype_ok(w->dtype) && (w->dtype != CPX_DT_F32 || !w->fuse_ln));
    const int dt = w->dtype, M = nS * 1024;
    const NetWs L = cpx_net_ws(nS, dt);
    CPX_REQUIRE(workspace_bytes >= L.total);
    char *ws = (char *)workspace;
    void *x = ws + L.off_x, *nk = ws + L.off_neck, *nk2 = ws + L.off_neck2;
    float *st = (float *)(ws + L.off_st);
    const CpxBlockBufs t = {x, x, x, ws + L.off_xn, ws + L.off_qkv, ws + L.off_vt, ws + L.off_ao, ws + L.off_h, st};
    CpxProf *prof = (CpxProf *)w->prof;
    if (prof) prof->phase = (prof->phase + 1) % prof->stride;
    hipStream_t hs = (hipStream_t)stream;
    const bool big_stats = cpx_net_big_stats(w, nS);
    const bool pe_stats = big_stats && cpx_gemm_half_uses_big_tile(M, 1024, 192, CPX_EPI_POS_BF16);
    TIMED(CPX_PROF_PE, 0, pe_stats ? cpx_gemm_half(dt, patches, w->pe_w, M, 1024, 192, CPX_EPI_POS_BF16, w->pe_b, w->pos, x, 1024, nullptr, nullptr, st, stream)
                                   : cpx_gemm(dt, patches, w->pe_w, M, 1024, 192, CPX_EPI_POS_BF16, w->pe_b, w->pos, x, 1024, stream));
    if (w->fuse_ln && !pe_stats) CPX_RUN(cpx_row_stats_half(dt, x, M, st, stream));
    for (int i = 0; i < w->depth; ++i) CPX_RUN(cpx_net_block(w, i, nS, t, big_stats, prof, stream));
    TIMED(CPX_PROF_TAIL, 0, cpx_net_tail(w, x, nS, nk, nk2, nk, nk2, ws + L.off_col, head, ws + L.total, workspace_bytes - L.total, stream));
    return CPX_OK;
}
#undef TIMED

template <int ES>
__global__ void __launch_bounds__(256) k_conv_gather(const char *__restrict__ a, int lda, int ca,
                                                     const char *__restrict__ b, int ldb, int cb,
                                                     int kind, int h, int w, size_t rows_out, int kpad,
                                                     char *__restrict__ out) {
    constexpr int EPC = 16 / ES;
    const int ctot = ca + cb, ccn = ctot / EPC, taps = kind == 0 ? 9 : (kind == 1 ? 4 : 1);
    const int chunks_per_row = kpad / EPC;
    size_t i = (size_t)blockIdx.x * 256 + threadIdx.x;
    if (i >= rows_out * chunks_per_row) return;
    size_t row = i / chunks_per_row;
    int ch = (int)(i - row * chunks_per_row);
    uint4 v = make_uint4(0, 0, 0, 0);
    const int ho = kind == 1 ? h >> 1 : h, wo = kind == 1 ? w >> 1 : w;
    if (ch < taps * ccn) {
        int tap = ch / ccn, cc = ch - tap * ccn;
        size_t s_ = row / (size_t)(ho * wo);
        int t = (int)(row - s_ * ho * wo), y = t / wo, x = t - y * wo;
        int yy, xx;
        if (kind == 0) { yy = y + tap / 3 - 1; xx = x + tap % 3 - 1; }
        else if (kind == 1) { yy = 2 * y + (tap >> 1); xx = 2 * x + (tap & 1); }
        else { yy = y; xx = x; }
        if ((unsigned)yy < (unsigned)h && (unsigned)xx < (unsigned)w) {
            size_t src_row = s_ * h * w + (size_t)yy * w + xx;
            int c = cc * EPC;
            v = c < ca ? *reinterpret_cast<const uint4 *>(a + (src_row * lda + c) * ES)
                       : *reinterpret_cast<const uint4 *>(b + (src_row * ldb + (c - ca)) * ES);
        }
    }
    *reinterpret_cast<uint4 *>(out + (row * kpad + (size_t)ch * EPC) * ES) = v;
}

template <int DT>
__global__ void __launch_bounds__(256) k_depth2space(const char *__restrict__ in, int ld_in, int cout,
                                                     int h, int w, size_t rows_in, char *__restrict__ out,
                                                     int ld_out, float *__restrict__ out_f32, int ld_f32, int col0) {
    constexpr int ES = DT == CPX_DT_F32 ? 4 : 2, EPC = 16 / ES;
    const int ccn = cout / EPC;
    size_t i = (size_t)blockIdx.x * 256 + threadIdx.x;
    if (i >= rows_in * 4 * ccn) return;
    size_t row = i / (4 * ccn);
    int rem = (int)(i - row * 4 * ccn), tap = rem / ccn, cc = rem - tap * ccn;
    size_t s_ = row / (size_t)(h * w);
    int t = (int)(row - s_ * h * w), y = t / w, x = t - y * w;
    size_t orow = s_ * 4 * h * w + (size_t)(2 * y + (tap >> 1)) * (2 * w) + 2 * x + (tap & 1);
    uint4 v = *reinterpret_cast<const uint4 *>(in + (row * ld_in + tap * cout + cc * EPC) * ES);
    if (out_f32) {
        float *o = out_f32 + orow * ld_f32 + col0 + cc * EPC;
        if constexpr (DT == CPX_DT_F32) {
            *reinterpret_cast<uint4 *>(o) = v;
        } else {
            const unsigned u[4] = {v.x, v.y, v.z, v.w};
#pragma unroll
            for (int k = 0; k < 4; ++k) { o[2 * k] = f32_from_h<DT == CPX_DT_F16>(u[k] & 0xFFFF); o[2 * k + 1] = f32_from_h<DT == CPX_DT_F16>(u[k] >> 16); }
        }
    } else {
        *reinterpret_cast<uint4 *>(out + (orow * ld_out + cc * EPC) * ES) = v;
    }
}

struct UnetLayout {
    size_t col_off, g_off, total;
    size_t off[64];
    int ld[64];
};
static void unet_layout(int dtype, const cpx_conv_op *ops, int n_ops, int nS, UnetLayout &L) {
    const size_t es = es_of(dtype);
    size_t col_max = 0, g_max = 0;
    for (int i = 0; i < n_ops; ++i) {
        const OpDims d = op_dims(ops[i], nS);
        col_max = std::max(col_max, (size_t)d.rows_pad * d.Kpad * es);
        if (ops[i].kind == 2) g_max = std::max(g_max, (size_t)d.rows_pad * d.Npad * es);
    }
    CpxArena a;
    L.col_off = a.take(col_max);
    L.g_off = a.take(g_max);
    for (int i = 0; i < n_ops && i < 64; ++i) {
        const OpDims d = op_dims(ops[i], nS);
        L.ld[i] = d.ld;
        L.off[i] = a.take((size_t)d.rows_out_pad * d.ld * es);
    }
    L.total = a.o + 1024;
}

size_t cpx_unet_ws_bytes(int dtype, const cpx_conv_op *ops, int n_ops, int nS) {
    if (!ops || n_ops <= 0 || n_ops > 64 || nS <= 0) return 0;
    UnetLayout L;
    unet_layout(dtype, ops, n_ops, nS, L);
    return L.total;
}
extern "C" size_t cpx_unet_workspace_bytes(const cpx_conv_op *ops, int n_ops, int nS, int dtype) {
    return cpx_unet_ws_bytes(dtype, ops, n_ops, nS);
}
void cpx_unet_act_layout(int dtype, const cpx_conv_op *ops, int n_ops, int nS, size_t *off, int *ld) {
    UnetLayout L;
    unet_layout(dtype, ops, n_ops, nS, L);
    for (int i = 0; i < n_ops && i < 64; ++i) { off[i] = L.off[i]; ld[i] = L.ld[i]; }
}
#ifdef CPX_DEBUG
extern "C" int cpx_unet_head_layout(const cpx_conv_op *ops, int n_ops, int nS, int dtype, size_t *dst_off, int *ld) {
    CPX_REQUIRE(ops && n_ops > 0 && n_ops <= 64 && nS > 0 && dst_off && ld && ops[n_ops - 1].kind == 2);
    UnetLayout L;
    unet_layout(dtype, ops, n_ops, nS, L);
    for (int i = 0; i < n_ops; ++i) { dst_off[i] = L.off[i]; ld[i] = L.ld[i]; }
    dst_off[n_ops - 1] = L.g_off;
    ld[n_ops - 1] = op_dims(ops[n_ops - 1], nS).Npad;
    return CPX_OK;
}
#endif

int cpx_unet_head_run(int dtype, const cpx_conv_op *ops, int n_ops, const void *feat, int nS, float *head,
                      int ld_head, int col0, void *workspace, size_t ws_bytes, void *stream) {
    CPX_REQUIRE(ops && n_ops > 0 && n_ops <= 64 && feat && head && workspace && nS > 0);
    CPX_REQUIRE(ws_bytes >= cpx_unet_ws_bytes(dtype, ops, n_ops, nS));
    hipStream_t s = (hipStream_t)stream;
    const size_t es = es_of(dtype);
    CpxTensor tens[66];
    tens[0] = {(const char *)feat, 256, 256, 32, 32};
    char *ws = (char *)workspace;
    UnetLayout lay;
    unet_layout(dtype, ops, n_ops, nS, lay);
    char *colbuf = ws + lay.col_off, *gbuf = ws + lay.g_off;
    const auto gather = es == 4 ? k_conv_gather<4> : k_conv_gather<2>;
    auto d2s = k_depth2space<CPX_DT_F32>;
    if (dtype != CPX_DT_F32) d2s = dtype == CPX_DT_F16 ? k_depth2space<CPX_DT_F16> : k_depth2space<CPX_DT_BF16>;
    for (int i = 0; i < n_ops; ++i) {
        const cpx_conv_op &o = ops[i];
        CPX_REQUIRE(o.dst > 0 && o.dst < 66 && o.src_a >= 0 && o.src_a < 66 && o.src_b < 66);
        CPX_REQUIRE(o.cin_a % 8 == 0 && o.cin_b % 8 == 0 && o.cout % 8 == 0 && o.weight && o.bias);
        const CpxTensor &A = tens[o.src_a];
        const CpxTensor Bz = {nullptr, 0, 0, 0, 0};
        const CpxTensor &B = o.src_b >= 0 ? tens[o.src_b] : Bz;
        CPX_REQUIRE(A.c == o.cin_a && A.h == o.h && A.w == o.w && (o.src_b < 0 || (B.c == o.cin_b && B.h == o.h && B.w == o.w)));
        if (o.kind == 2) CPX_REQUIRE(o.src_b < 0);
        const OpDims d = op_dims(o, nS);
        const bool convT = o.kind == 2;
        const dim3 grid_g((unsigned)((d.rows * (d.Kpad / (16 / es)) + 255) / 256));
        hipLaunchKernelGGL(gather, grid_g, dim3(256), 0, s, A.p, A.ld, o.cin_a, B.p, B.ld, convT ? 0 : o.cin_b, convT ? 3 : o.kind, o.h, o.w, d.rows, d.Kpad, colbuf);
        char *dst = ws + lay.off[i];
        const int rc = cpx_gemm(dtype, colbuf, o.weight, d.rows_pad, d.Npad, d.Kpad, !convT && o.relu ? CPX_EPI_RELU_BF16 : CPX_EPI_BF16, o.bias, nullptr,
                                convT ? gbuf : dst, d.Npad, stream);
        if (rc) return rc;
        if (convT) {
            const bool last = i == n_ops - 1;
            const dim3 grid((unsigned)((d.rows * 4 * (o.cout / (16 / es)) + 255) / 256));
            hipLaunchKernelGGL(d2s, grid, dim3(256), 0, s, gbuf, d.Npad, o.cout, o.h, o.w, d.rows, dst, d.ld, last ? head : nullptr, ld_head, col0);
        }
        tens[o.dst] = {dst, d.ld, o.cout, d.ho, d.wo};
    }
    CPX_CHECK_LAUNCH();
    return CPX_OK;
}
// ... 5 lines not shown
```

classpose_amd/csrc/cpx_pre.hip:

```cpp
#include "cpx_common.h"

#define NTHR 256

__device__ __forceinline__ void cv_linear_tap(int d, double scale, int slen, bool clamp_weight,
                                              int &s0, int &s1, int &w0, int &w1) {
    float f = (float)(((double)d + 0.5) * scale - 0.5);
    int s = (int)floorf(f);
    f -= (float)s;
    if (clamp_weight) {
        if (s < 0) { f = 0.f; s = 0; }
        if (s >= slen - 1) { f = 0.f; s = slen - 1; }
    }
    w0 = __float2int_rn((1.f - f) * 2048.f);
    w1 = __float2int_rn(f * 2048.f);
    s0 = min(max(s, 0), slen - 1);
    s1 = min(max(s + 1, 0), slen - 1);
}

__global__ void k_resize_linear_u8(const uint8_t *__restrict__ src, int sh, int sw,
                                   uint8_t *__restrict__ dst, int dh, int dw, double scale_x,
                                   double scale_y, int area2) {
    int p = blockIdx.x * NTHR + threadIdx.x;
    if (p >= dh * dw) return;
    int dy = p / dw, dx = p - dy * dw;
// ... 168 lines not shown
    return *reinterpret_cast<unsigned short *>(&h);
}
template <int DT>
__global__ void k_make_patches(const uint8_t *__restrict__ tiles, const float *__restrict__ stats,
                               TilingDev g, void *__restrict__ patches_v) {
    const int tok_per = (g.b / 8) * (g.b / 8);
    const int per_sub = tok_per * 24;
    int i = blockIdx.x * NTHR + threadIdx.x;
    if (i >= per_sub) return;
    int sub = blockIdx.y;
    int t = sub / (g.ny * g.nx), ji = sub - t * g.ny * g.nx;
    int j = ji / g.nx, ii_t = ji - j * g.nx;
    int tok = i / 24, r = i - tok * 24;
    int c = r >> 3, ii = r & 7;
    int ph = tok / (g.b / 8), pw = tok - ph * (g.b / 8);
    bool fy = g.augment && (ii_t & 1) && !(j & 1);
    bool fx = g.augment && (j & 1) && !(ii_t & 1);
    if (g.augment && (j & 1) && (ii_t & 1)) { fy = true; fx = true; }
    int y = 8 * ph + ii;
    int sy = fy ? g.b - 1 - y : y;
    union { unsigned short h[8]; uint4 v; } o;
    float f[8];
#pragma unroll
    for (int jj = 0; jj < 8; ++jj) {
        int x = 8 * pw + jj;
        int sx = fx ? g.b - 1 - x : x;
        float v = padded_px(tiles, stats, g, t, g.ys[j] + sy, g.xs[ii_t] + sx, c);
        f[jj] = v;
        o.h[jj] = DT == 1 ? f32_to_f16(v) : f32_to_bf16(v);
    }
    const size_t e = ((size_t)sub * tok_per + tok) * 192 + c * 64 + ii * 8;
    if constexpr (DT == 2) {
        float *patches = (float *)patches_v;
        *reinterpret_cast<float4 *>(patches + e) = make_float4(f[0], f[1], f[2], f[3]);
        *reinterpret_cast<float4 *>(patches + e + 4) = make_float4(f[4], f[5], f[6], f[7]);
    } else {
        *reinterpret_cast<uint4 *>((unsigned short *)patches_v + e) = o.v;
    }
}

__global__ void k_make_subtiles_f32(const uint8_t *__restrict__ tiles, const float *__restrict__ stats,
                                    TilingDev g, float *__restrict__ out) {
    int i = blockIdx.x * NTHR + threadIdx.x;
    int per = 3 * g.b * g.b;
    if (i >= per) return;
    int sub = blockIdx.y;
    int t = sub / (g.ny * g.nx), ji = sub - t * g.ny * g.nx;
    int j = ji / g.nx, ii_t = ji - j * g.nx;
    int c = i / (g.b * g.b), r = i - c * g.b * g.b;
    int y = r / g.b, x = r - y * g.b;
    bool fy = g.augment && (ii_t & 1) && !(j & 1);
    bool fx = g.augment && (j & 1) && !(ii_t & 1);
    if (g.augment && (j & 1) && (ii_t & 1)) { fy = true; fx = true; }
    int sy = fy ? g.b - 1 - y : y, sx = fx ? g.b - 1 - x : x;
    out[(size_t)sub * per + i] = padded_px(tiles, stats, g, t, g.ys[j] + sy, g.xs[ii_t] + sx, c);
}

extern "C" int cpx_make_patches(const uint8_t *tiles, const float *stats, int nT,
                                const cpx_tiling *tiling, int dtype, void *patches, void *stream) {
    TilingDev g; int rc = tiling_to_dev(tiling, &g); if (rc) return rc;
    CPX_REQUIRE(tiles && stats && patches && nT > 0 && dtype >= 0 && dtype <= 2);
    int per_sub = (g.b / 8) * (g.b / 8) * 24;
    const dim3 grid(cpx_cdiv(per_sub, NTHR), nT * g.ny * g.nx);
    if (dtype == 2) hipLaunchKernelGGL(k_make_patches<2>, grid, dim3(NTHR), 0, (hipStream_t)stream, tiles, stats, g, patches);
    else if (dtype == 1) hipLaunchKernelGGL(k_make_patches<1>, grid, dim3(NTHR), 0, (hipStream_t)stream, tiles, stats, g, patches);
    else hipLaunchKernelGGL(k_make_patches<0>, grid, dim3(NTHR), 0, (hipStream_t)stream, tiles, stats, g, patches);
    CPX_CHECK_LAUNCH();
    return CPX_OK;
}
extern "C" int cpx_make_subtiles(const uint8_t *tiles, const float *stats, int nT,
                                 const cpx_tiling *tiling, void *patches, void *stream) {
    return cpx_make_patches(tiles, stats, nT, tiling, 0, patches, stream);
}

extern "C" int cpx_make_subtiles_f32(const uint8_t *tiles, const float *stats, int nT,
                                     const cpx_tiling *tiling, float *subtiles, void *stream) {
    TilingDev g; int rc = tiling_to_dev(tiling, &g); if (rc) return rc;
    CPX_REQUIRE(tiles && stats && subtiles && nT > 0);
    hipLaunchKernelGGL(k_make_subtiles_f32, dim3(cpx_cdiv(3 * g.b * g.b, NTHR), nT * g.ny * g.nx),
                       dim3(NTHR), 0, (hipStream_t)stream, tiles, stats, g, subtiles);
    CPX_CHECK_LAUNCH();
    return CPX_OK;
}

template <bool TOKEN_MAJOR>
__global__ void k_blend(const float *__restrict__ src, const float *__restrict__ src2, int ld, int ncls,
                        TilingDev g, const double *__restrict__ taper, float *__restrict__ dP,
                        float *__restrict__ cellprob, float *__restrict__ logits) {
    int idx = blockIdx.x * NTHR + threadIdx.x;
    const int HW = g.H * g.W;
    if (idx >= HW) return;
    const int ch = blockIdx.z;
    size_t t = blockIdx.y;
    int Y = idx / g.W, X = idx - Y * g.W;
    int Yp = Y + g.ypad1, Xp = X + g.xpad1;
    const int tb = g.b / 8;
    float acc = 0.f;
    double navg = 0.0;
    for (int j = 0; j < g.ny; ++j) {
        int y = Yp - g.ys[j];
        if ((unsigned)y >= (unsigned)g.b) continue;
        for (int i = 0; i < g.nx; ++i) {
            int x = Xp - g.xs[i];
            if ((unsigned)x >= (unsigned)g.b) continue;
            bool fy = g.augment && (i & 1) && !(j & 1);
            bool fx = g.augment && (j & 1) && !(i & 1);
            if (g.augment && (j & 1) && (i & 1)) { fy = true; fx = true; }
            int sy = fy ? g.b - 1 - y : y, sx = fx ? g.b - 1 - x : x;
            size_t sub = (t * g.ny + j) * g.nx + i;
            float v;
            if (TOKEN_MAJOR) {
                int tok = (sy >> 3) * tb + (sx >> 3);
                int col = (ch < 3 ? ch * 64 : 192 + (ch - 3) * 64) + (sy & 7) * 8 + (sx & 7);
                v = src[(sub * tb * tb + tok) * (size_t)ld + col];
            } else {
                v = ch < 3 ? src[((sub * 3 + ch) * g.b + sy) * (size_t)g.b + sx]
                           : src2[((sub * ncls + (ch - 3)) * g.b + sy) * (size_t)g.b + sx];
            }
            if ((ch == 0 && fy) || (ch == 1 && fx)) v = -v;
            double m = taper[x] * taper[y];
            acc = (float)((double)acc + (double)v * m);
            navg = navg + m;
        }
    }
    float r = (float)((double)acc / navg);
    if (ch < 2) dP[(t * 2 + ch) * HW + idx] = r;
    else if (ch == 2) cellprob[t * HW + idx] = r;
    else logits[(t * ncls + (ch - 3)) * HW + idx] = r;
}

extern "C" int cpx_blend_subtiles(const float *head, int ld_head, int ncls, int nT,
                                  const cpx_tiling *tiling, const double *taper1d, float *dP,
                                  float *cellprob, float *logits, void *stream) {
    TilingDev g; int rc = tiling_to_dev(tiling, &g); if (rc) return rc;
    CPX_REQUIRE(head && taper1d && dP && cellprob && nT > 0 && ncls >= 0 && (ncls == 0 || logits));
    CPX_REQUIRE(ld_head >= 192 + ncls * 64);
    hipLaunchKernelGGL(k_blend<true>, dim3(cpx_cdiv(g.H * g.W, NTHR), nT, 3 + ncls), dim3(NTHR), 0,
                       (hipStream_t)stream, head, (const float *)nullptr, ld_head, ncls, g, taper1d,
                       dP, cellprob, logits);
    CPX_CHECK_LAUNCH();
    return CPX_OK;
}

extern "C" int cpx_blend_subtiles_nchw(const float *y, const float *y_class, int ncls, int nT,
                                       const cpx_tiling *tiling, const double *taper1d, float *dP,
                                       float *cellprob, float *logits, void *stream) {
    TilingDev g; int rc = tiling_to_dev(tiling, &g); if (rc) return rc;
    CPX_REQUIRE(y && taper1d && dP && cellprob && nT > 0 && ncls >= 0 && (ncls == 0 || (logits && y_class)));
    hipLaunchKernelGGL(k_blend<false>, dim3(cpx_cdiv(g.H * g.W, NTHR), nT, 3 + ncls), dim3(NTHR), 0,
                       (hipStream_t)stream, y, y_class, 0, ncls, g, taper1d, dP, cellprob, logits);
    CPX_CHECK_LAUNCH();
    return CPX_OK;
}
```

classpose_amd/engine.py:

```python
from __future__ import annotations

import os

import ctypes as C
import math
from dataclasses import dataclass

import numpy as np
import torch

from . import _lib
from ._lib import CpxBlockWeights, CpxConvOp, CpxNetWeights, CpxRecord, CpxTiling, check, ptr

PS = 8
BSIZE = 256
HALF_DTYPES = {"bf16": torch.bfloat16, "fp16": torch.float16}
NET_DTYPES = {**HALF_DTYPES, "fp32": torch.float32}


def make_tiling(H: int, W: int, bsize: int = BSIZE, augment: bool = False,
                tile_overlap: float = 0.1) -> CpxTiling:
    def pad(L):
        lpad = int(16 * math.ceil(L / 16) - L) if L >= bsize else bsize - L
        return 8 + lpad // 2, 8 + lpad - lpad // 2
# ... 194 lines not shown
        self.fts = fts
        if jobs:
            with torch.cuda.device(dev):
                stage = torch.empty(stage_bytes, dtype=torch.uint8, device=dev)
                arr = (_lib.CpxWeightJob * len(jobs))(*jobs)
                st = torch.cuda.current_stream(dev)
                check(L.cpx_weights_build(arr, len(jobs), stage.data_ptr(), stage_bytes, st.cuda_stream), "weights_build")
                st.synchronize()
                del stage
        sources.clear()
        return self

    def _build_unet_ops(self, sd, fts, out_ch, half, vec32):
        hd = {0: torch.bfloat16, 1: torch.float16, 2: torch.float32}[self.c.dtype]
        up = lambda x, m: (x + m - 1) // m * m
        p8 = lambda c: up(c, 8)
        ops = []

        def rounded(t):
            return t.detach().to(hd).float()

        def add(kind, src_a, src_b, cin_a, cin_b, cout, h, relu, wkey):
            w, b = rounded(sd[wkey + ".weight"]), rounded(sd[wkey + ".bias"])
            ca, cb, co = p8(cin_a), p8(cin_b), p8(cout)
            if kind == 2:
                wt = torch.zeros(2, 2, co, ca)
                wt[:, :, :cout, :cin_a] = w.permute(2, 3, 1, 0)
                wm = wt.reshape(4 * co, ca)
                bt = torch.zeros(4, co)
                bt[:, :cout] = b[None, :]
                bm = bt.reshape(-1)
            else:
                k = w.shape[-1]
                wt = torch.zeros(co, k, k, ca + cb)
                wk = w.permute(0, 2, 3, 1)
                wt[:cout, :, :, :cin_a] = wk[..., :cin_a]
                wt[:cout, :, :, ca:ca + cin_b] = wk[..., cin_a:]
                wm = wt.reshape(co, -1)
                bm = torch.zeros(co)
                bm[:cout] = b
            n_pad, k_pad = up(wm.shape[0], 128), up(wm.shape[1], 64)
            wp = torch.zeros(n_pad, k_pad)
            wp[: wm.shape[0], : wm.shape[1]] = wm
            bp = torch.zeros(n_pad)
            bp[: bm.shape[0]] = bm
            op = CpxConvOp()
            op.kind, op.src_a, op.src_b, op.dst = kind, src_a, src_b, len(ops) + 1
            op.cin_a, op.cin_b, op.cout, op.h, op.w, op.relu = ca, cb, co, h, h, int(relu)
            op.weight, op.bias = half(wp), vec32(bp)
            ops.append(op)
            return op.dst

        def block(pfx, src_a, src_b, cin_a, cin_b, cout, h, last_relu=True):
            t = add(0, src_a, src_b, cin_a, cin_b, cout, h, True, pfx + "block.conv1")
            return add(0, t, -1, cout, 0, cout, h, last_relu, pfx + "block.conv2")

        cur, cin, h, feats = 0, 256, 32, []
        for n, c in enumerate(fts):
            p = f"out_class.encoder_blocks.{n}."
            t = block(p, cur, -1, cin, 0, c, h)
            cur = add(1, t, -1, c, 0, c, h, False, p + "downconv")
            h //= 2
            feats.append((cur, c))
            cin = c
        c = fts[-1]
        t = block("out_class.bottleneck_down.", cur, -1, c, 0, c, h)
        cur = add(1, t, -1, c, 0, c, h, False, "out_class.bottleneck_down.downconv")
        h //= 2
        t = block("out_class.bottleneck_up.", cur, -1, c, 0, c, h)
        cur = add(2, t, -1, c, 0, c, h, False, "out_class.bottleneck_up.upconv")
        h *= 2
        seq = [*fts[::-1], out_ch]
        feats = feats[::-1]
        for i in range(len(fts)):
            p = f"out_class.decoder_blocks.{i}."
            fid, fc = feats[i]
            t = block(p, cur, fid, seq[i], fc, seq[i + 1], h, last_relu=(i != len(fts) - 1))
            cur = add(2, t, -1, seq[i + 1], 0, seq[i + 1], h, False, p + "upconv")
            h *= 2
        if h != 32:
            raise ValueError(f"UNet head: {len(fts)} levels do not end on the 32 x 32 token grid (reached {h})")
        if out_ch % 8 != 0:
            raise ValueError(f"UNet head: out_ch = {out_ch} is not a multiple of 8")
        self.unet_ops = (CpxConvOp * len(ops))(*ops)
        self.c.n_unet_ops = len(ops)
        self.c.unet_ops = C.cast(self.unet_ops, C.POINTER(CpxConvOp))


@dataclass
class TileOutputs:
    masks: torch.Tensor
    class_masks: torch.Tensor
    nlabels: torch.Tensor
    dP: torch.Tensor
    cellprob: torch.Tensor
    logits: torch.Tensor | None
    records: torch.Tensor | None = None
    rec_counts: torch.Tensor | None = None
    cells: torch.Tensor | None = None
    xy_pool: torch.Tensor | None = None
    n_pts_total: torch.Tensor | None = None
    votes: torch.Tensor | None = None
    prob_q: torch.Tensor | None = None
    cellprob_q: torch.Tensor | None = None


class _Slot:

    def __init__(self, eng: "Engine"):
        nT, H, W, ncls, d = eng.nT, eng.nH, eng.nW, eng.w.ncls, eng.dev
        cH, cW = eng.cH, eng.cW
        nS = nT * eng.n_sub
        self.stats = torch.empty(nT * 3 * 4, dtype=torch.float32, device=d)
        self.hist = torch.empty(nT * 768, dtype=torch.int32, device=d)
        self.patches = torch.zeros(nS * 1024 * 192 * (2 if eng.w.c.dtype == _lib.DT_F32 else 1), dtype=torch.int16, device=d)
        self.head = torch.empty(nS * 1024 * eng.w.c.ld_head, dtype=torch.float32, device=d)
        self.dP = torch.empty((nT, 2, H, W), dtype=torch.float32, device=d)
        self.cellprob = torch.empty((nT, H, W), dtype=torch.float32, device=d)
        self.logits = torch.empty((nT, max(ncls, 1), H, W), dtype=torch.float32, device=d)
        self.pp_ws = torch.empty(eng.pp_ws_bytes, dtype=torch.uint8, device=d)
        self.masks = torch.empty((nT, cH, cW), dtype=torch.int16, device=d)
        self.class_masks = torch.empty((nT, cH, cW), dtype=torch.uint8, device=d)
        self.nlabels = torch.empty(nT, dtype=torch.int32, device=d)
        self.records = torch.empty(nT * eng.max_rec * C.sizeof(CpxRecord), dtype=torch.uint8, device=d)
        self.rec_counts = torch.empty(nT, dtype=torch.int32, device=d)
        self.cells = self.xy_pool = self.n_pts_total = self.poly_ws = self.origins = None
        self.has_polygons = False
        self.votes = self.prob_q = self.cellprob_q = None
        self.has_confidence = False
        if eng.rescaled:
            tH, tW = eng.H, eng.W
            self.tiles_net = torch.empty((nT, H, W, 3), dtype=torch.uint8, device=d)
            self.out_dP = torch.empty((nT, 2, tH, tW), dtype=torch.float32, device=d)
            self.out_cellprob = torch.empty((nT, tH, tW), dtype=torch.float32, device=d)
            self.out_logits = torch.empty((nT, max(ncls, 1), tH, tW), dtype=torch.float32, device=d)
            if not eng.resample:
                self.out_masks = torch.empty((nT, tH, tW), dtype=torch.int16, device=d)
                self.out_class_masks = torch.empty((nT, tH, tW), dtype=torch.uint8, device=d)
        self.ev_net = torch.cuda.Event()
        self.ev_post = torch.cuda.Event()
        self.n = 0
        self.inject = None
        self.busy = False


class Engine:

    N_SLOTS = 2

    def __init__(self, weights: NetWeights, tile_h: int = 256, tile_w: int | None = None,
                 batch_tiles: int = 8, augment: bool = False, tile_overlap: float = 0.1,
                 niter: int = 200, cellprob_threshold: float = 0.0, flow_threshold: float = 0.4,
                 min_size: int = 15, max_size_fraction: float = 0.4, net_hw: tuple[int, int] | None = None,
                 resample: bool = True):
        self.L = _lib.lib()
        self.w = weights
        self.dev = weights.device
        self.H, self.W = tile_h, tile_w or tile_h
        self.nT = batch_tiles
        self.nH, self.nW = (int(net_hw[0]), int(net_hw[1])) if net_hw is not None else (self.H, self.W)
        if self.nH < 1 or self.nW < 1:
            raise ValueError(f"Engine: net_hw = {net_hw} must be at least 1 x 1")
        self.rescaled = (self.nH, self.nW) != (self.H, self.W)
        self.resample = bool(resample) or not self.rescaled
        self.cH, self.cW = (self.H, self.W) if self.resample else (self.nH, self.nW)
        self.tiling = make_tiling(self.nH, self.nW, BSIZE, augment, tile_overlap)
        self.n_sub = self.tiling.ny * self.tiling.nx
        self.niter, self.cp_thr, self.flow_thr = niter, cellprob_threshold, flow_threshold
        self.min_size, self.max_frac = min_size, max_size_fraction
        nT, H, W = self.nT, self.cH, self.cW
        d = self.dev
        lo = percentile_params(self.nH * self.nW, 1)
        hi = percentile_params(self.nH * self.nW, 99)
        self.pct = (lo[0], lo[1], hi[0], hi[1])
        self.net_ws_bytes = self.L.cpx_net_workspace_bytes(nT * self.n_sub, weights.c.dtype)
        if weights.c.n_unet_ops:
            self.net_ws_bytes += self.L.cpx_unet_workspace_bytes(weights.c.unet_ops, weights.c.n_unet_ops,
                                                                nT * self.n_sub, weights.c.dtype)
        self.net_ws = torch.empty(self.net_ws_bytes, dtype=torch.uint8, device=d)
        self.taper = torch.from_numpy(taper_1d(BSIZE)).to(d)
        self.pp_ws_bytes = self.L.cpx_postproc_workspace_bytes(nT, H, W)
        self.max_rec = min(self.L.cpx_postproc_max_labels(H, W), 65535)
        self.max_pts = nT * max(4096, 2 * H * W)
        self.slots = [_Slot(self) for _ in range(self.N_SLOTS)]
        self.s_net = torch.cuda.Stream(d, priority=int(os.environ.get("CPX_NET_STREAM_PRIORITY", "0")))
        self.s_post = torch.cuda.Stream(d, priority=int(os.environ.get("CPX_POST_STREAM_PRIORITY", "0")))
        self._next = 0
        self._last: _Slot | None = None
        self.stage_timing: list | None = None

    def submit(self, tiles_u8: torch.Tensor, inject=None, records: bool = True, polygons=None, confidence: bool = False) -> int:
        if tiles_u8.dtype != torch.uint8 or tiles_u8.dim() != 4 or not tiles_u8.is_contiguous():
            raise ValueError(f"Engine.submit: tiles must be a contiguous uint8 [n, H, W, 3] tensor, got {tiles_u8.dtype} {tuple(tiles_u8.shape)}")
        n = tiles_u8.shape[0]
        if n > self.nT or tuple(tiles_u8.shape[1:]) != (self.H, self.W, 3):
            raise ValueError(f"Engine.submit: got {tuple(tiles_u8.shape)}, this engine takes at most {self.nT} tiles of {(self.H, self.W, 3)}")
        if tiles_u8.device != self.dev:
            raise ValueError(f"Engine.submit: tiles live on {tiles_u8.device}, the engine on {self.dev}")
        if self.rescaled and not self.resample and (records or polygons is not None):
            raise ValueError("Engine.submit: records / polygons of a resample=False engine would be in network-size coordinates; "
                             "pass records=False")
        if inject is not None:
            if len(inject) != 3 or inject[0] is None or inject[1] is None or (inject[2] is None and self.w.ncls > 1):
                raise ValueError("Engine.submit: inject = (dP, cellprob, logits) device tensors (logits may be None only without a class head)")
            if any(t is not None and (t.device != self.dev or not t.is_contiguous()) for t in inject):
                raise ValueError("Engine.submit: inject = (dP, cellprob, logits) contiguous tensors on the engine's device")
            if self.rescaled and any(t is not None and tuple(t.shape[-2:]) != (self.nH, self.nW) for t in inject):
                raise ValueError(f"Engine.submit: inject fields of this engine are at network size {(self.nH, self.nW)}")
        sid = self._next
        self._next = (self._next + 1) % self.N_SLOTS
        sl = self.slots[sid]
        if sl.busy:
            raise RuntimeError("Engine: slot still holds an uncollected batch; call result() first")
        sl.n, sl.inject, sl.busy = n, inject, True
        cur = torch.cuda.current_stream(self.dev)
        self.s_net.wait_stream(cur)
        self.s_net.wait_event(sl.ev_post)
        lo_p, lo_g, hi_p, hi_g = self.pct
        sn, sp = self.s_net.cuda_stream, self.s_post.cuda_stream
        tm = self.stage_timing
        ev = [torch.cuda.Event(enable_timing=True) for _ in range(5)] if tm is not None else None
        if ev:
            ev[0].record(self.s_net)
        src = tiles_u8
        if self.rescaled:
            check(self.L.cpx_resize_linear_u8(ptr(tiles_u8), n, self.H, self.W, ptr(sl.tiles_net), self.nH, self.nW, sn), "resize_linear_u8")
            src = sl.tiles_net
        check(self.L.cpx_normalize_stats_u8(ptr(src), n, self.nH, self.nW, lo_p, lo_g, hi_p, hi_g,
                                            ptr(sl.stats), ptr(sl.hist), sn), "normalize_stats")
        check(self.L.cpx_make_patches(ptr(src), ptr(sl.stats), n, C.byref(self.tiling), self.w.c.dtype,
                                      ptr(sl.patches), sn), "make_patches")
        if ev:
            ev[1].record(self.s_net)
        check(self.L.cpx_net_forward(C.byref(self.w.c), ptr(sl.patches), self.nT * self.n_sub, ptr(sl.head),
                                     ptr(self.net_ws), self.net_ws_bytes, sn), "net_forward")
        if ev:
            ev[2].record(self.s_net)
        sl.ev_net.record(self.s_net)
        tiles_u8.record_stream(self.s_net)
        self.s_post.wait_event(sl.ev_net)
        if inject is not None:
            self.s_post.wait_stream(cur)
        ncls = self.w.ncls
        if ev:
            ev[3].record(self.s_post)
        check(self.L.cpx_blend_subtiles(ptr(sl.head), self.w.c.ld_head, ncls if ncls > 1 else 0, n,
                                        C.byref(self.tiling), ptr(self.taper), ptr(sl.dP),
                                        ptr(sl.cellprob), ptr(sl.logits), sp), "blend")
        if ev:
            ev[4].record(self.s_post)
            tm.append(ev)
        dP, cp, lg = (sl.dP, sl.cellprob, sl.logits) if inject is None else inject
        if self.rescaled:
            for a, b, planes in ((dP, sl.out_dP, 2), (cp, sl.out_cellprob, 1), (lg, sl.out_logits, ncls if ncls > 1 else 0)):
                if planes:
                    check(self.L.cpx_resize_linear_f32(ptr(a), n * planes, self.nH, self.nW, ptr(b), self.H, self.W, sp), "resize_linear_f32")
            if self.resample:
                dP, cp, lg = sl.out_dP, sl.out_cellprob, sl.out_logits
        check(self.L.cpx_compute_masks_records(ptr(dP), ptr(cp), ptr(lg) if ncls > 1 else None, n, ncls,
                                               self.cH, self.cW, self.cp_thr, self.flow_thr, self.niter,
                                               self.min_size, self.max_frac, ptr(sl.masks), ptr(sl.class_masks),
                                               ptr(sl.nlabels), self.max_rec if records else 0,
                                               ptr(sl.records) if records else None, ptr(sl.rec_counts) if records else None,
                                               ptr(sl.pp_ws), sp), "compute_masks")
        sl.has_confidence = bool(confidence)
        if confidence:
            if sl.cellprob_q is None:
                if ncls > 1:
                    sl.votes = torch.empty((self.nT, self.max_rec, ncls), dtype=torch.int32, device=self.dev)
                    sl.prob_q = torch.empty((self.nT, self.max_rec, ncls), dtype=torch.int64, device=self.dev)
                sl.cellprob_q = torch.empty((self.nT, self.max_rec), dtype=torch.int64, device=self.dev)
                self.s_post.wait_stream(cur)
            check(self.L.cpx_instance_confidence(ptr(sl.masks), ptr(lg) if ncls > 1 else None, ptr(cp),
                                                 ptr(sl.rec_counts if records else sl.nlabels), n,
                                                 ncls, self.cH, self.cW, self.max_rec, ptr(sl.votes), ptr(sl.prob_q),
                                                 ptr(sl.cellprob_q), None, 0, sp), "instance_confidence")
        if self.rescaled and not self.resample:
            check(self.L.cpx_resize_nearest(ptr(sl.masks), 2, n, self.nH, self.nW, ptr(sl.out_masks), self.H, self.W, sp), "resize_nearest")
            check(self.L.cpx_resize_nearest(ptr(sl.class_masks), 1, n, self.nH, self.nW, ptr(sl.out_class_masks), self.H, self.W, sp),
                  "resize_nearest")
        sl.has_polygons = polygons is not None
        if polygons is not None:
            if not records:
                raise ValueError("Engine.submit: polygons need the per-cell records (records=True)")
            scale, origins = polygons
            if sl.cells is None:
                sl.cells = torch.empty(self.nT * self.max_rec * C.sizeof(_lib.CpxCell), dtype=torch.uint8, device=self.dev)
                sl.xy_pool = torch.empty((self.max_pts, 2), dtype=torch.float64, device=self.dev)
                sl.n_pts_total = torch.empty(1, dtype=torch.int32, device=self.dev)
                sl.poly_ws = torch.empty(self.L.cpx_polygonize_workspace_bytes(self.nT, self.H, self.W, self.max_rec),
                                         dtype=torch.uint8, device=self.dev)
                sl.origins_host = torch.zeros((self.nT, 2), dtype=torch.float64).pin_memory()
                sl.origins = torch.empty((self.nT, 2), dtype=torch.float64, device=self.dev)
                self.s_post.wait_stream(cur)
            sl.origins_host[:n] = torch.as_tensor(np.asarray(origins, dtype=np.float64).reshape(n, 2))
            with torch.cuda.stream(self.s_post):
                sl.origins.copy_(sl.origins_host, non_blocking=True)
            check(self.L.cpx_polygonize_device(ptr(sl.masks), ptr(sl.records), ptr(sl.rec_counts), n, self.H, self.W,
                                               self.max_rec, float(scale), ptr(sl.origins), ptr(sl.xy_pool),
                                               self.max_pts, ptr(sl.cells), ptr(sl.n_pts_total), ptr(sl.poly_ws), sp),
                  "polygonize_device")
        sl.ev_post.record(self.s_post)
        return sid

    def result(self, sid: int, wait: bool = True) -> "TileOutputs":
        sl = self.slots[sid]
        if wait:
            torch.cuda.current_stream(self.dev).wait_event(sl.ev_post)
        sl.busy = False
        self._last = sl
        n = sl.n
        masks, cm = (sl.masks, sl.class_masks) if self.resample else (sl.out_masks, sl.out_class_masks)
        dP, cp, lg = (sl.out_dP, sl.out_cellprob, sl.out_logits) if self.rescaled else (sl.dP, sl.cellprob, sl.logits)
        return TileOutputs(masks[:n], cm[:n], sl.nlabels[:n], dP[:n], cp[:n],
                           lg[:n] if self.w.ncls > 1 else None, sl.records, sl.rec_counts,
                           *((sl.cells, sl.xy_pool, sl.n_pts_total) if sl.has_polygons else (None, None, None)),
                           *((sl.votes, sl.prob_q, sl.cellprob_q) if sl.has_confidence else (None, None, None)))

    def run(self, tiles_u8: torch.Tensor, inject=None, records: bool = True, polygons=None, confidence: bool = False) -> "TileOutputs":
        return self.result(self.submit(tiles_u8, inject, records, polygons, confidence))

    def fetch_confidence(self, out: "TileOutputs", tile: np.ndarray, label: np.ndarray):
        ti = torch.as_tensor(np.asarray(tile, dtype=np.int64), device=self.dev)
        ri = torch.as_tensor(np.asarray(label, dtype=np.int64) - 1, device=self.dev)
        m = len(ti)
        cq = out.cellprob_q[ti, ri].cpu().numpy().view(np.uint64)
        if out.votes is None:
            return np.zeros((m, 0), np.int64), np.zeros((m, 0), np.uint64), cq
        return out.votes[ti, ri].cpu().numpy().astype(np.int64), out.prob_q[ti, ri].cpu().numpy().view(np.uint64), cq

    def fetch_polygons(self, n: int, out: "TileOutputs"):
        total = int(out.n_pts_total.item())
        if total > self.max_pts:
            return None
        counts = self._checked_counts(out.rec_counts, n)
        mx = int(counts.max()) if n else 0
        raw = out.cells.view(self.nT, self.max_rec, CELL_DTYPE.itemsize)[:n, :mx].cpu().numpy().view(CELL_DTYPE).reshape(n, mx)
        rows = [raw[t, :int(counts[t])] for t in range(n)]
        tile = np.concatenate([np.full(len(r), t, np.int32) for t, r in enumerate(rows)]) if n else np.zeros(0, np.int32)
        cells = np.concatenate(rows) if n else raw[:0, 0]
        return cells, tile, out.xy_pool[:total].cpu().numpy()

    @property
    def records(self):
        return self._last.records

    @property
    def rec_counts(self):
        return self._last.rec_counts

    def fetch_records(self, n: int, out: "TileOutputs | None" = None) -> np.ndarray:
        recs = self._last.records if out is None else out.records
        cnts = self._last.rec_counts if out is None else out.rec_counts
        counts = self._checked_counts(cnts, n)
        mx = int(counts.max()) if n else 0
        raw = recs.view(self.nT, self.max_rec, RECORD_DTYPE.itemsize)[:n, :mx].cpu().numpy().view(RECORD_DTYPE).reshape(n, mx)
        return np.concatenate([raw[t, :int(counts[t])] for t in range(n)]) if n else raw.reshape(-1)

    def _checked_counts(self, rec_counts: torch.Tensor, n: int) -> np.ndarray:
        counts = rec_counts[:n].cpu().numpy()
        if n and int(counts.max()) > self.max_rec:
            raise RuntimeError(f"a tile holds {int(counts.max())} instances but the record buffer has {self.max_rec} "
                               "slots per tile: cells would be dropped")
        return counts


CELL_DTYPE = np.dtype([("area", "<f8"), ("perimeter", "<f8"), ("cx", "<f8"), ("cy", "<f8"),
                       ("n_pts", "<i4"), ("offset", "<i4"), ("valid", "<i4"), ("cls", "<i4")])
assert CELL_DTYPE.itemsize == C.sizeof(_lib.CpxCell)
RECORD_DTYPE = np.dtype([("tile", "<i4"), ("label", "<i4"), ("cls", "<i4"), ("area", "<i4"),
                         ("y0", "<i4"), ("x0", "<i4"), ("y1", "<i4"), ("x1", "<i4"),
                         ("sum_y", "<i8"), ("sum_x", "<i8")])
assert RECORD_DTYPE.itemsize == C.sizeof(CpxRecord)
```

include/classpose_hip.h:

```cpp
#ifndef CLASSPOSE_HIP_H
#define CLASSPOSE_HIP_H

#include <stddef.h>
#include <stdint.h>

#ifdef __cplusplus
extern "C" {
#endif

#define CPX_OK 0
#define CPX_EINVAL (-22)
#define CPX_ENOMEM (-12)
#define CPX_EHIP (-5)

#define CPX_DT_BF16 0
#define CPX_DT_F16 1
#define CPX_DT_F32 2

int cpx_abi_version(void);
const char *cpx_last_error(void);
const char *cpx_build_id(void);

int cpx_normalize_stats_u8(const uint8_t *tiles_u8, int nT, int H, int W,
                           int lo_prev, float lo_gamma, int hi_prev, float hi_gamma,
                           float *stats, uint32_t *hist_ws, void *stream);
int cpx_normalize_apply_u8(const uint8_t *tiles_u8, const float *stats, int nT, int H, int W,
                           float *out_f32, void *stream);

int cpx_resize_linear_u8(const uint8_t *src_u8, int nT, int sh, int sw,
                         uint8_t *dst_u8, int dh, int dw, void *stream);

typedef struct cpx_tiling {
    int H, W;
    int ypad1, xpad1;
    int Ly, Lx;
    int ny, nx;
    int bsize;
    int augment;
    int ystart[16];
    int xstart[16];
} cpx_tiling;

int cpx_make_subtiles(const uint8_t *tiles_u8, const float *stats, int nT,
                      const cpx_tiling *tiling_host, void *patches_bf16, void *stream);
int cpx_make_patches(const uint8_t *tiles_u8, const float *stats, int nT,
                     const cpx_tiling *tiling_host, int dtype, void *patches, void *stream);
int cpx_make_subtiles_f32(const uint8_t *tiles_u8, const float *stats, int nT,
                          const cpx_tiling *tiling_host, float *subtiles, void *stream);
int cpx_blend_subtiles(const float *head, int ld_head, int ncls, int nT,
                       const cpx_tiling *tiling_host, const double *taper1d,
                       float *dP, float *cellprob, float *logits, void *stream);
int cpx_blend_subtiles_nchw(const float *y, const float *y_class, int ncls, int nT,
                            const cpx_tiling *tiling_host, const double *taper1d,
                            float *dP, float *cellprob, float *logits, void *stream);

typedef struct cpx_block_weights {
    const float *ln1_w, *ln1_b;
    const void *qkv_w;  const float *qkv_b;
    const void *proj_w; const float *proj_b;
    const void *rel_h, *rel_w;
    const float *ln2_w, *ln2_b;
    const void *fc1_w;  const float *fc1_b;
    const void *fc2_w;  const float *fc2_b;
    const float *qkv_colsum, *fc1_colsum;
} cpx_block_weights;

typedef struct cpx_conv_op {
    int kind;
    int src_a, src_b;
    int dst;
    int cin_a, cin_b, cout;
    int h, w;
    int relu;
    const void *weight;
    const float *bias;
} cpx_conv_op;

typedef struct cpx_net_weights {
    int depth;
    int ncls;
    int n_head_cols;
    int ld_head;
    int dtype;
    int fuse_ln;
    const void *pe_w;
    const float *pe_b;
    const float *pos;
    const cpx_block_weights *blocks;
    const void *neck0_w;
    const float *neck_ln1_w, *neck_ln1_b;
    const void *neck2_w;
    const float *neck_ln2_w, *neck_ln2_b;
    const void *head_w;
    const float *head_b;
    int n_unet_ops;
    const cpx_conv_op *unet_ops;
    void *prof;
} cpx_net_weights;

int cpx_round_weights(const float *src, void *dst, long long n, int dtype, int keep_f32, void *stream);
int cpx_fold_layernorm(const float *w, const float *b, const float *gamma, const float *beta, int N, int K, int dtype,
                       void *w_folded, float *b_folded, float *colsum, void *stream);
#define CPX_WJ_ROUND_HALF 0
#define CPX_WJ_ROUND_F32 1
#define CPX_WJ_COPY_F32 2
#define CPX_WJ_FOLD_LN 3
typedef struct cpx_weight_job {
    int op;
    int dtype;
    long long n;
    int K;
    int reserved;
    const void *src_host[4];
    size_t stage_off[4];
    void *dst[3];
} cpx_weight_job;
int cpx_weights_build(const cpx_weight_job *jobs_host, int n_jobs, void *stage_base, size_t stage_bytes, void *stream);

size_t cpx_net_workspace_bytes(int n_subtiles, int dtype);
size_t cpx_unet_workspace_bytes(const cpx_conv_op *ops_host, int n_ops, int n_subtiles, int dtype);
int cpx_unet_head_forward(const cpx_conv_op *ops_host, int n_ops, const void *feat, int n_subtiles,
                          float *head, int ld_head, int col0, int dtype, void *workspace,
                          size_t workspace_bytes, void *stream);
int cpx_net_mlp_parts(int n_subtiles, int dtype);
int cpx_net_forward(const cpx_net_weights *w_host, const void *patches, int n_subtiles,
                    float *head, void *workspace, size_t workspace_bytes, void *stream);

#define CPX_PROF_N_KINDS 7
int cpx_prof_create(int max_launches, int stride, unsigned kinds_mask, void **prof_out);
int cpx_prof_collect(void *prof, double *ms_sum, int *count);
int cpx_prof_collect_launches(void *prof, float *ms, int *kind, int cap, int *n_out);
void cpx_prof_destroy(void *prof);

typedef struct cpx_qc_op {
    int kind, k, stride, pad, act;
    int h_in, w_in, h_out, w_out;
    size_t src_a, src_b, gate, res, dst;
    int c_a, ld_a, up_a, c_b, ld_b, ld_res, c_out, ld_dst, c_red;
    const float *w, *bias, *w2, *bias2;
} cpx_qc_op;
int cpx_qc_forward(const cpx_qc_op *ops_host, int n_ops, const uint8_t *patches_u8, int nB, int H, int W,
                   size_t input_off, size_t logits_off, int n_classes, int ld_logits,
                   int8_t *class_map, float *logits_out, void *workspace, size_t workspace_bytes,
                   void *stream);

#define CPX_EPI_BF16 0
#define CPX_EPI_GELU_BF16 1
#define CPX_EPI_RESID_BF16 2
#define CPX_EPI_F32 3
#define CPX_EPI_POS_BF16 4
#define CPX_EPI_RELU_BF16 5
#define CPX_EPI_QKV_BF16 6
int cpx_gemm_bf16(const void *A, const void *Wt, int M, int N, int K, int epilogue,
                  const float *bias, const void *resid_or_pos, void *out, int ld_out,
                  void *stream);
int cpx_gemm(int dtype, const void *A, const void *Wt, int M, int N, int K, int epilogue,
             const float *bias, const void *resid_or_pos, void *out, int ld_out, void *stream);

int cpx_conv3x3(int dtype, const void *x, const void *Wt, int M, int N, int C, int epilogue, const float *bias,
                void *out, int ld_out, void *stream);
int cpx_gemm_uses_big_tile(int M, int N, int K, int epilogue);
int cpx_gemm_ln(const void *A, const void *Wt, int M, int N, int K, int epilogue,
                const float *bias, const void *resid_or_pos, void *out, int ld_out,
                const float *ln_stats, const float *ln_colsum, float *stats_out, void *stream);
int cpx_row_stats(const void *x, int rows, float *stats, void *stream);
int cpx_layernorm_bf16(const void *x, const float *w, const float *b, int rows, int C,
                       float eps, void *out, void *stream);
int cpx_attention_relpos(const void *qkv, const void *rel_h, const void *rel_w, int n_subtiles,
                         void *vT_ws, void *out, void *stream);
int cpx_layernorm(int dtype, const void *x, const float *w, const float *b, int rows, int C,
                  float eps, void *out, void *stream);
int cpx_attention(int dtype, const void *qkv, const void *rel_h, const void *rel_w, int n_subtiles,
                  void *vT_ws, void *out, void *stream);

size_t cpx_postproc_workspace_bytes(int nT, int H, int W);
int cpx_postproc_max_labels(int H, int W);
unsigned long long cpx_postproc_launch_count(void);

int cpx_follow_flows(const float *dP, const float *cellprob, int nT, int H, int W,
                     float cellprob_threshold, int niter, int32_t *p_final, float *p_float,
                     void *workspace, void *stream);
int cpx_get_masks(const int32_t *p_final, int nT, int H, int W, double max_size_fraction,
                  int32_t *masks, int32_t *nlabels, void *workspace, void *stream);
int cpx_remove_bad_flow_masks(int32_t *masks, const float *dP, int nT, int H, int W,
                              double threshold, double *flow_errors, void *workspace,
                              void *stream);
int cpx_fill_holes_and_remove_small_masks(int32_t *masks, int nT, int H, int W, int min_size,
                                          int32_t *nlabels, void *workspace, void *stream);
int cpx_compute_class_masks(const int32_t *masks, const float *logits, int nT, int ncls, int H,
                            int W, uint8_t *class_masks, void *workspace, void *stream);
int cpx_remove_border_instances(int32_t *masks, uint8_t *class_masks, int nT, int H, int W,
                                void *workspace, void *stream);
int cpx_compute_masks(const float *dP, const float *cellprob, const float *logits, int nT,
                      int ncls, int H, int W, float cellprob_threshold, double flow_threshold,
                      int niter, int min_size, double max_size_fraction, uint16_t *masks_u16,
                      uint8_t *class_masks, int32_t *nlabels, void *workspace, void *stream);


typedef struct cpx_record {
    int32_t tile;
    int32_t label;
    int32_t cls;
    int32_t area;
    int32_t y0, x0, y1, x1;
    int64_t sum_y, sum_x;
} cpx_record;
int cpx_instance_records(const uint16_t *masks_u16, const uint8_t *class_masks, int nT, int H,
                         int W, int max_records_per_tile, cpx_record *records,
                         int32_t *counts, void *workspace, void *stream);
int cpx_compute_masks_records(const float *dP, const float *cellprob, const float *logits, int nT,
                              int ncls, int H, int W, float cellprob_threshold,
                              double flow_threshold, int niter, int min_size,
                              double max_size_fraction, uint16_t *masks_u16,
                              uint8_t *class_masks, int32_t *nlabels, int max_rec, cpx_record *records,
                              int32_t *rec_counts, void *workspace, void *stream);

size_t cpx_instance_confidence_workspace_bytes(int nT, int ncls, int H, int W, int max_rec);
int cpx_instance_confidence(const uint16_t *masks_u16, const float *logits, const float *cellprob,
                            const int32_t *rec_counts, int nT, int ncls, int H, int W, int max_rec,
                            int32_t *votes, uint64_t *prob_q, uint64_t *cellprob_q,
                            void *workspace, size_t workspace_bytes, void *stream);

int cpx_resize_linear_f32(const float *src, int n_planes, int sh, int sw, float *dst, int dh, int dw, void *stream);
int cpx_resize_nearest(const void *src, int elem_bytes, int n_planes, int sh, int sw, void *dst, int dh, int dw,
                       void *stream);

typedef struct cpx_pq_pair {
    int32_t image, cls;
    int32_t first_true, first_pred;
    int32_t inter, area_true, area_pred, reserved;
} cpx_pq_pair;
typedef struct cpx_pq_inst {
    int32_t image, side, cls;
    int32_t first, area, reserved;
} cpx_pq_inst;
size_t cpx_pq_workspace_bytes(int nI, int H, int W, int nr_classes, int table_cap);
int cpx_pq_stats(const void *true_ids, const void *pred_ids, int id_bytes, const uint8_t *true_cls, const uint8_t *pred_cls,
                 int nI, int H, int W, int nr_classes, double match_iou, int filter_unlabelled, int no_border_instances,
                 int table_cap, int32_t *tp, int32_t *fp, int32_t *fn, double *iou_sum, int32_t *status, int32_t *nobg,
                 cpx_pq_pair *pairs, int max_pairs, cpx_pq_inst *insts, int max_insts, int32_t *list_counts,
                 void *workspace, size_t workspace_bytes, void *stream);

size_t cpx_net_neck_offset(int n_subtiles, int dtype);
int cpx_patchify_f32(const float *x, int nS, int H, int W, int dtype, void *patches, void *stream);

#define CPX_LOSS_EMPTY_IMAGE 1
#define CPX_LOSS_BAD_LABEL 2
size_t cpx_class_loss_workspace_bytes(int nI, int H, int W, int ncls);
int cpx_class_loss(const float *head, int ld_head, int col0, const int16_t *labels, int nI, int H, int W, int ncls,
                   const float *class_weights, float alpha, float gamma, float eps, float w_ce, float w_tv,
                   float *ce, float *tversky, float *tp, float *fp, float *fn, int32_t *n_annot, float *dlogits,
                   int32_t *status, void *workspace, size_t workspace_bytes, void *stream);

int cpx_head_wgrad_slab_rows(void);
size_t cpx_head_wgrad_workspace_bytes(int rows, int n_cols);
int cpx_head_wgrad(const float *dlogits, const void *feat, int dtype, int rows, int n_cols, float *dW, float *db,
                   void *workspace, size_t workspace_bytes, void *stream);

int cpx_adamw_step(float *param, const float *grad, float *exp_avg, float *exp_avg_sq, long long n, double lr,
                   double beta1, double beta2, double eps, double weight_decay, double bias_correction1,
                   double bias_correction2, void *stream);

int cpx_unet_wgrad_slab_rows(void);
long long cpx_unet_param_layout(const cpx_conv_op *ops_host, int n_ops, long long *w_off, long long *b_off, int *n_pad, int *k_pad);
int cpx_unet_refresh_operands(const cpx_conv_op *ops_host, int n_ops, const float *params, int dtype, void *stream);
size_t cpx_unet_backward_workspace_bytes(const cpx_conv_op *ops_host, int n_ops, int n_subtiles, int dtype);
int cpx_unet_grad_layout(const cpx_conv_op *ops_host, int n_ops, int n_subtiles, int dtype, size_t *g_off, int *g_ld);
int cpx_unet_head_backward(const cpx_conv_op *ops_host, int n_ops, const void *feat, int n_subtiles, int dtype,
                           const void *fwd_workspace, size_t fwd_workspace_bytes, const float *dlogits, float *grads,
                           void *workspace, size_t workspace_bytes, void *stream);

size_t cpx_net_backbone_offset(int n_subtiles, int dtype);
size_t cpx_neck_train_workspace_bytes(int n_subtiles, int dtype);
int cpx_neck_train_layout(int n_subtiles, int dtype, size_t *off );
int cpx_neck_forward_train(const cpx_net_weights *w, const void *x, int n_subtiles, float *head, void *workspace,
                           size_t workspace_bytes, void *stream);
size_t cpx_layernorm_backward_workspace_bytes(int rows, int C);
int cpx_layernorm_backward(int dtype, const void *y, const float *gamma, const float *dout, int rows, int C, float eps,
                           float *dy, float *dgamma, float *dbeta, void *workspace, size_t workspace_bytes, void *stream);
long long cpx_neck_grad_layout(long long *off );
size_t cpx_neck_backward_workspace_bytes(int n_subtiles, int dtype, int ld_head, size_t *off );
int cpx_neck_backward(const cpx_net_weights *w, const void *x, int n_subtiles, const void *fwd_workspace, size_t fwd_workspace_bytes,
                      const float *dhead, float *grads, void *workspace, size_t workspace_bytes, void *stream);

size_t cpx_blocks_train_workspace_bytes(int n_subtiles, int dtype, int n_blocks);
int cpx_blocks_train_layout(int n_subtiles, int dtype, int n_blocks, size_t *off );
int cpx_blocks_forward_train(const cpx_net_weights *w, const void *x, int n_subtiles, int first_block, float *head, void *workspace,
                             size_t workspace_bytes, void *stream);
long long cpx_block_grad_layout(long long *off );
size_t cpx_blocks_backward_workspace_bytes(int n_subtiles, int dtype);
int cpx_blocks_backward_slab_crops(void);
int cpx_blocks_backward(const cpx_net_weights *w, const float *params, int n_subtiles, int first_block, const void *fwd_workspace,
                        size_t fwd_workspace_bytes, const float *dy0, float *grads, float *dx_all, void *workspace,
                        size_t workspace_bytes, void *stream);
size_t cpx_blocks_backward_workspace_bytes_ex(int n_subtiles, int dtype, int grad_dtype);
int cpx_blocks_backward_ex(const cpx_net_weights *w, const float *params, int n_subtiles, int first_block, const void *fwd_workspace,
                           size_t fwd_workspace_bytes, const float *dy0, int grad_dtype, float *grads, float *dx_all, void *workspace,
                           size_t workspace_bytes, void *stream);
int cpx_gemm_tn_bf16(const void *A, const void *B, int M, int N, int K, int add, float *out, int ld_out, void *stream);
size_t cpx_colsum_workspace_bytes(int rows, int N);
int cpx_colsum_add(const float *dy, int rows, int N, float *db, void *workspace, size_t workspace_bytes, void *stream);
size_t cpx_layernorm_backward_bytes(int rows, int C);
size_t cpx_attention_backward_workspace_bytes(int n_subtiles);
int cpx_attention_backward(int dtype, const void *qkv, const void *rel_h, const void *rel_w, const void *O, const float *dO,
                           int n_subtiles, float *dqkv, float *drel_h, float *drel_w, void *workspace, size_t workspace_bytes,
// ... 152 lines not shown
```

Baseline: 366.8 tiles/s.

## Write head GEMM output as per-subtile channel planes and blend via precomputed tap table

Result: no change. 367.3 tiles/s (median of 6 runs) (+0.1%).

```diff
diff --git a/classpose_amd/_lib.py b/classpose_amd/_lib.py
--- a/classpose_amd/_lib.py
+++ b/classpose_amd/_lib.py
@@ -97,12 +97,16 @@
     "cpx_make_subtiles_f32": (_i, [_p, _p, _i, C.POINTER(CpxTiling), _p, _p]),
     "cpx_blend_subtiles": (_i, [_p, _i, _i, _i, C.POINTER(CpxTiling), _p, _p, _p, _p, _p]),
     "cpx_blend_subtiles_nchw": (_i, [_p, _p, _i, _i, C.POINTER(CpxTiling), _p, _p, _p, _p, _p]),
+    "cpx_blend_table_bytes": (_sz, [C.POINTER(CpxTiling)]),
+    "cpx_blend_table_build": (_i, [C.POINTER(CpxTiling), _p, _p, _sz, _p]),
+    "cpx_blend_planes": (_i, [_p, _i, _i, C.POINTER(CpxTiling), _p, _sz, _p, _p, _p, _p]),
     "cpx_qc_forward": (_i, [C.POINTER(CpxQcOp), _i, _p, _i, _i, _i, _sz, _sz, _i, _i, _p, _p, _p, _sz, _p]),
     "cpx_round_weights": (_i, [_p, _p, C.c_longlong, _i, _i, _p]),
     "cpx_fold_layernorm": (_i, [_p, _p, _p, _p, _i, _i, _i, _p, _p, _p, _p]),
     "cpx_weights_build": (_i, [C.POINTER(CpxWeightJob), _i, _p, _sz, _p]),
     "cpx_net_workspace_bytes": (_sz, [_i, _i]),
     "cpx_net_forward": (_i, [C.POINTER(CpxNetWeights), _p, _i, _p, _p, _sz, _p]),
+    "cpx_net_forward_planes": (_i, [C.POINTER(CpxNetWeights), _p, _i, _p, _p, _sz, _p]),
     "cpx_unet_workspace_bytes": (_sz, [C.POINTER(CpxConvOp), _i, _i, _i]),
     "cpx_unet_head_forward": (_i, [C.POINTER(CpxConvOp), _i, _p, _i, _p, _i, _i, _i, _p, _sz, _p]),
     "cpx_net_mlp_parts": (_i, [_i, _i]),
diff --git a/classpose_amd/csrc/cpx_gemm.hip b/classpose_amd/csrc/cpx_gemm.hip
--- a/classpose_amd/csrc/cpx_gemm.hip
+++ b/classpose_amd/csrc/cpx_gemm.hip
@@ -43,6 +43,7 @@
     const float *ln_colsum;
     float *stats_out;
     int conv_c;
+    int n_planes;
 };
 #define LN_SLOTS 4
 __device__ __forceinline__ float2 ln_mean_rstd(float4 a, float4 b, float inv_k) {
@@ -253,6 +254,13 @@
             }
             if constexpr (EPI == CPX_EPI_F32) {
                 *reinterpret_cast<float4 *>((float *)g.out + (size_t)m * g.ld_out + n) = make_float4(v[0], v[1], v[2], v[3]);
+            } else if constexpr (EPI == CPX_EPI_F32_PLANES) {
+                const int c = n >> 6;
+                if (c < g.n_planes) {
+                    const size_t s_ = (size_t)(m >> 10);
+                    const int py = ((m >> 5) & 31) * 8 + ((n >> 3) & 7), px = (m & 31) * 8 + (n & 7);
+                    *reinterpret_cast<float4 *>((float *)g.out + ((s_ * g.n_planes + c) * 256 + py) * 256 + px) = make_float4(v[0], v[1], v[2], v[3]);
+                }
             } else if (EPI == CPX_EPI_QKV_BF16 && n >= 2048) {
                 unsigned short *vT = (unsigned short *)g.aux;
                 const size_t s_ = (size_t)(m >> 10), t_ = (size_t)(m & 1023);
@@ -933,7 +941,7 @@
 }
 
 int cpx_gemm_half_uses_big_tile(int M, int N, int K, int epilogue) {
-    if (epilogue == CPX_EPI_F32) return 0;
+    if (epilogue == CPX_EPI_F32 || epilogue == CPX_EPI_F32_PLANES) return 0;
     if (!g_gemm_big || M % 256 || N % 256 || K < 128) return 0;
     if ((K / 64) % 2 && epilogue != CPX_EPI_POS_BF16) return 0;
     return (M / 256) * (N / 256) >= 256;
@@ -969,7 +977,7 @@
 
 template <int EPI, bool F16>
 static bool launch_gemm256(const GemmArgs &a0, hipStream_t s) {
-    if constexpr (EPI == CPX_EPI_F32) return false;
+    if constexpr (EPI == CPX_EPI_F32 || EPI == CPX_EPI_F32_PLANES) return false;
     else {
         if (!cpx_gemm_half_uses_big_tile(a0.M, a0.N, a0.K, EPI)) return false;
         GemmArgs a = a0;
@@ -1104,7 +1112,8 @@
     CPX_REQUIRE(A && Wt && out && (dtype == CPX_DT_BF16 || dtype == CPX_DT_F16));
     const bool f16 = dtype == CPX_DT_F16;
     CPX_REQUIRE(M > 0 && N > 0 && K > 0 && M % BM == 0 && N % BN == 0 && K % BK == 0);
-    CPX_REQUIRE(ld_out >= N && ld_out % 4 == 0);
+    const bool planes = epilogue == CPX_EPI_F32_PLANES;
+    CPX_REQUIRE(planes ? (ld_out > 0 && ld_out * 64 <= N && M % 1024 == 0) : (ld_out >= N && ld_out % 4 == 0));
     CPX_REQUIRE((epilogue != CPX_EPI_RESID_BF16 && epilogue != CPX_EPI_POS_BF16 && epilogue != CPX_EPI_QKV_BF16) || aux);
     CPX_REQUIRE(epilogue != CPX_EPI_QKV_BF16 || (N == 3072 && M % 1024 == 0));
     CPX_REQUIRE(!ln_stats || (ln_colsum && epilogue != CPX_EPI_RESID_BF16));
@@ -1112,6 +1121,7 @@
     GemmArgs a = gemm_args(A, Wt, M, N, K, bias, aux, out, ld_out);
     a.ln_stats = ln_stats; a.ln_colsum = ln_colsum; a.stats_out = stats_out; a.l2_block = g_gemm_l2; a.nt_out = g_gemm_nt;
     a.rev_m = (g_gemm_rev && K >= 4096) ? 1 : 0;
+    if (planes) a.n_planes = ld_out;
     hipStream_t s = (hipStream_t)stream;
     switch (epilogue) {
         case CPX_EPI_BF16: launch_gemm<CPX_EPI_BF16>(a, s, f16); break;
@@ -1121,6 +1131,7 @@
         case CPX_EPI_POS_BF16: launch_gemm<CPX_EPI_POS_BF16>(a, s, f16); break;
         case CPX_EPI_RELU_BF16: launch_gemm<CPX_EPI_RELU_BF16>(a, s, f16); break;
         case CPX_EPI_QKV_BF16: launch_gemm<CPX_EPI_QKV_BF16>(a, s, f16); break;
+        case CPX_EPI_F32_PLANES: launch_gemm<CPX_EPI_F32_PLANES>(a, s, f16); break;
         default: CPX_REQUIRE(!"unknown epilogue");
     }
     CPX_CHECK_LAUNCH();
diff --git a/classpose_amd/csrc/cpx_internal.h b/classpose_amd/csrc/cpx_internal.h
--- a/classpose_amd/csrc/cpx_internal.h
+++ b/classpose_amd/csrc/cpx_internal.h
@@ -78,7 +78,7 @@
 int cpx_net_block(const cpx_net_weights *w, int layer, int nS, const CpxBlockBufs &t, bool big_stats, CpxProf *prof, void *stream);
 bool cpx_net_big_stats(const cpx_net_weights *w, int nS);
 int cpx_net_tail(const cpx_net_weights *w, const void *x, int nS, void *y0, void *a1, void *y2, void *feat, void *col, float *head,
-                 void *unet_ws, size_t unet_ws_bytes, void *stream);
+                 void *unet_ws, size_t unet_ws_bytes, void *stream, bool head_planes = false);
 
 int cpx_unet_head_run(int dtype, const cpx_conv_op *ops, int n_ops, const void *feat, int nS, float *head, int ld_head,
                       int col0, void *workspace, size_t ws_bytes, void *stream);
diff --git a/classpose_amd/csrc/cpx_net.hip b/classpose_amd/csrc/cpx_net.hip
--- a/classpose_amd/csrc/cpx_net.hip
+++ b/classpose_amd/csrc/cpx_net.hip
@@ -467,8 +467,9 @@
 }
 
 int cpx_net_tail(const cpx_net_weights *w, const void *x, int nS, void *y0, void *a1, void *y2, void *feat, void *col, float *head,
-                 void *unet_ws, size_t unet_ws_bytes, void *stream) {
+                 void *unet_ws, size_t unet_ws_bytes, void *stream, bool head_planes) {
     const int dt = w->dtype, M = nS * 1024;
+    CPX_REQUIRE(!head_planes || (dt != CPX_DT_F32 && w->n_unet_ops == 0 && w->n_head_cols % 64 == 0));
     CPX_RUN(cpx_gemm(dt, x, w->neck0_w, M, 256, 1024, CPX_EPI_BF16, nullptr, nullptr, y0, 256, stream));
     CPX_RUN(cpx_layernorm(dt, y0, w->neck_ln1_w, w->neck_ln1_b, M, 256, 1e-6f, a1, stream));
     if (dt == CPX_DT_F32) {
@@ -478,7 +479,8 @@
         CPX_RUN(cpx_conv3_half(dt, a1, w->neck2_w, M, 256, 256, CPX_EPI_BF16, nullptr, y2, 256, stream));
     }
     CPX_RUN(cpx_layernorm(dt, y2, w->neck_ln2_w, w->neck_ln2_b, M, 256, 1e-6f, feat, stream));
-    CPX_RUN(cpx_gemm(dt, feat, w->head_w, M, w->ld_head, 256, CPX_EPI_F32, w->head_b, nullptr, head, w->ld_head, stream));
+    if (head_planes) CPX_RUN(cpx_gemm(dt, feat, w->head_w, M, w->ld_head, 256, CPX_EPI_F32_PLANES, w->head_b, nullptr, head, w->n_head_cols / 64, stream));
+    else CPX_RUN(cpx_gemm(dt, feat, w->head_w, M, w->ld_head, 256, CPX_EPI_F32, w->head_b, nullptr, head, w->ld_head, stream));
     if (w->n_unet_ops > 0) {
         const size_t need = cpx_unet_ws_bytes(dt, w->unet_ops, w->n_unet_ops, nS);
         CPX_REQUIRE(unet_ws_bytes >= need);
@@ -532,8 +534,8 @@
     return CPX_OK;
 }
 
-extern "C" int cpx_net_forward(const cpx_net_weights *w, const void *patches, int nS, float *head,
-                               void *workspace, size_t workspace_bytes, void *stream) {
+static int net_forward(const cpx_net_weights *w, const void *patches, int nS, float *head,
+                       void *workspace, size_t workspace_bytes, void *stream, bool head_planes) {
     CPX_REQUIRE(w && patches && head && workspace && nS > 0);
     CPX_REQUIRE(w->depth > 0 && w->blocks && w->ld_head % 128 == 0 && w->ld_head >= w->n_head_cols);
     CPX_REQUIRE(dtype_ok(w->dtype) && (w->dtype != CPX_DT_F32 || !w->fuse_ln));
@@ -553,10 +555,19 @@
                                    : cpx_gemm(dt, patches, w->pe_w, M, 1024, 192, CPX_EPI_POS_BF16, w->pe_b, w->pos, x, 1024, stream));
     if (w->fuse_ln && !pe_stats) CPX_RUN(cpx_row_stats_half(dt, x, M, st, stream));
     for (int i = 0; i < w->depth; ++i) CPX_RUN(cpx_net_block(w, i, nS, t, big_stats, prof, stream));
-    TIMED(CPX_PROF_TAIL, 0, cpx_net_tail(w, x, nS, nk, nk2, nk, nk2, ws + L.off_col, head, ws + L.total, workspace_bytes - L.total, stream));
+    TIMED(CPX_PROF_TAIL, 0, cpx_net_tail(w, x, nS, nk, nk2, nk, nk2, ws + L.off_col, head, ws + L.total, workspace_bytes - L.total, stream, head_planes));
     return CPX_OK;
 }
 #undef TIMED
+extern "C" int cpx_net_forward(const cpx_net_weights *w, const void *patches, int nS, float *head,
+                               void *workspace, size_t workspace_bytes, void *stream) {
+    return net_forward(w, patches, nS, head, workspace, workspace_bytes, stream, false);
+}
+extern "C" int cpx_net_forward_planes(const cpx_net_weights *w, const void *patches, int nS, float *planes,
+                                      void *workspace, size_t workspace_bytes, void *stream) {
+    CPX_REQUIRE(w && w->dtype != CPX_DT_F32 && w->n_unet_ops == 0);
+    return net_forward(w, patches, nS, planes, workspace, workspace_bytes, stream, true);
+}
 
 template <int ES>
 __global__ void __launch_bounds__(256) k_conv_gather(const char *__restrict__ a, int lda, int ca,
diff --git a/classpose_amd/csrc/cpx_pre.hip b/classpose_amd/csrc/cpx_pre.hip
--- a/classpose_amd/csrc/cpx_pre.hip
+++ b/classpose_amd/csrc/cpx_pre.hip
@@ -344,3 +344,227 @@
     CPX_CHECK_LAUNCH();
     return CPX_OK;
 }
+
+#define BT_FY (1 << 16)
+#define BT_FX (1 << 17)
+#define BT_VEC (1 << 18)
+#define BT_QUAD (1 << 19)
+struct BlendTable {
+    int K;
+    size_t off_navg, off_m, off_tap, total;
+};
+static int blend_table_layout(const cpx_tiling *t, BlendTable *L) {
+    TilingDev g; int rc = tiling_to_dev(t, &g); if (rc) return rc;
+    CPX_REQUIRE(g.H > 0 && g.W > 0 && g.ny * g.nx <= 0xFFFF && (long long)g.b * g.b < (1ll << 31));
+    auto most = [&](int n, int pad, const int *start, int cnt) {
+        int best = 0;
+        for (int p = 0; p < n; ++p) {
+            int c = 0;
+            for (int j = 0; j < cnt; ++j) c += (unsigned)(p + pad - start[j]) < (unsigned)g.b;
+            best = c > best ? c : best;
+        }
+        return best;
+    };
+    L->K = most(g.H, g.ypad1, g.ys, g.ny) * most(g.W, g.xpad1, g.xs, g.nx);
+    if (L->K < 1) L->K = 1;
+    const size_t HW = (size_t)g.H * g.W;
+    CpxArena a;
+    L->off_navg = a.take(HW * sizeof(double));
+    L->off_m = a.take(HW * L->K * sizeof(double));
+    L->off_tap = a.take(HW * L->K * sizeof(int2));
+    L->total = a.o;
+    return CPX_OK;
+}
+
+__global__ void k_blend_table(TilingDev g, const double *__restrict__ taper, int K, double *__restrict__ navg_o,
+                              double *__restrict__ m_o, int2 *__restrict__ tap_o) {
+    int idx = blockIdx.x * NTHR + threadIdx.x;
+    const int HW = g.H * g.W;
+    if (idx >= HW) return;
+    int Y = idx / g.W, X = idx - Y * g.W;
+    int Yp = Y + g.ypad1, Xp = X + g.xpad1;
+    double navg = 0.0;
+    int k = 0;
+    for (int j = 0; j < g.ny; ++j) {
+        int y = Yp - g.ys[j];
+        if ((unsigned)y >= (unsigned)g.b) continue;
+        for (int i = 0; i < g.nx; ++i) {
+            int x = Xp - g.xs[i];
+            if ((unsigned)x >= (unsigned)g.b) continue;
+            bool fy = g.augment && (i & 1) && !(j & 1);
+            bool fx = g.augment && (j & 1) && !(i & 1);
+            if (g.augment && (j & 1) && (i & 1)) { fy = true; fx = true; }
+            int sy = fy ? g.b - 1 - y : y, sx = fx ? g.b - 1 - x : x;
+            double m = taper[x] * taper[y];
+            navg = navg + m;
+            if (k < K) {
+                tap_o[(size_t)k * HW + idx] = make_int2(sy * g.b + sx, (j * g.nx + i) | (fy ? BT_FY : 0) | (fx ? BT_FX : 0));
+                m_o[(size_t)k * HW + idx] = m;
+            }
+            ++k;
+        }
+    }
+    for (; k < K; ++k) {
+        tap_o[(size_t)k * HW + idx] = make_int2(0, -1);
+        m_o[(size_t)k * HW + idx] = 0.0;
+    }
+    navg_o[idx] = navg;
+}
+__global__ void k_blend_table_hints(TilingDev g, int K, int2 *__restrict__ tap) {
+    int q = blockIdx.x * NTHR + threadIdx.x;
+    const int HW = g.H * g.W;
+    if (q >= HW / 4) return;
+    const int idx = q * 4;
+    bool quad = true;
+    for (int k = 0; k < K; ++k) {
+        const int c0 = tap[(size_t)k * HW + idx].y;
+        for (int p = 1; p < 4; ++p) quad = quad && tap[(size_t)k * HW + idx + p].y == c0;
+    }
+    if (!quad) return;
+    for (int k = 0; k < K; ++k) {
+        int2 e = tap[(size_t)k * HW + idx];
+        if (e.y < 0) break;
+        const int lo = (e.y & BT_FX) ? e.x - 3 : e.x;
+        if ((lo & 3) == 0) e.y |= BT_VEC;
+        if (k == 0) e.y |= BT_QUAD;
+        tap[(size_t)k * HW + idx] = e;
+    }
+}
+
+template <int CH>
+__global__ void __launch_bounds__(NTHR) k_blend_planes(const float *__restrict__ planes, int C, int ncls, TilingDev g, int K,
+                                                       const double *__restrict__ navg_t, const double *__restrict__ m_t,
+                                                       const int2 *__restrict__ tap_t, float *__restrict__ dP,
+                                                       float *__restrict__ cellprob, float *__restrict__ logits) {
+    const int qw = (g.W + 3) >> 2;
+    const int q = blockIdx.x * NTHR + threadIdx.x;
+    if (q >= g.H * qw) return;
+    const int Y = q / qw, X0 = (q - Y * qw) * 4;
+    const int HW = g.H * g.W, idx0 = Y * g.W + X0;
+    const int npx = min(4, g.W - X0);
+    const size_t t = blockIdx.y, bb = (size_t)g.b * g.b;
+    const int c0 = blockIdx.z * CH;
+    const float *src = planes + t * g.ny * g.nx * C * bb;
+    float acc[CH][4];
+#pragma unroll
+    for (int cc = 0; cc < CH; ++cc)
+#pragma unroll
+        for (int p = 0; p < 4; ++p) acc[cc][p] = 0.f;
+    const int2 e0 = tap_t[idx0];
+    if (e0.y >= 0 && (e0.y & BT_QUAD)) {
+        for (int k = 0; k < K; ++k) {
+            const int2 e = tap_t[(size_t)k * HW + idx0];
+            if (e.y < 0) break;
+            const bool fy = e.y & BT_FY, fx = e.y & BT_FX;
+            const double2 ma = *reinterpret_cast<const double2 *>(m_t + (size_t)k * HW + idx0);
+            const double2 mb = *reinterpret_cast<const double2 *>(m_t + (size_t)k * HW + idx0 + 2);
+            const double m[4] = {ma.x, ma.y, mb.x, mb.y};
+            const float *s = src + (size_t)(e.y & 0xFFFF) * C * bb;
+            const int step = fx ? -1 : 1;
+            float v[CH][4];
+#pragma unroll
+            for (int cc = 0; cc < CH; ++cc) {
+                if (c0 + cc >= C) break;
+                const float *sc = s + (size_t)(c0 + cc) * bb + e.x;
+                if (e.y & BT_VEC) {
+                    const float4 f = *reinterpret_cast<const float4 *>(fx ? sc - 3 : sc);
+                    v[cc][0] = fx ? f.w : f.x; v[cc][1] = fx ? f.z : f.y; v[cc][2] = fx ? f.y : f.z; v[cc][3] = fx ? f.x : f.w;
+                } else {
+#pragma unroll
+                    for (int p = 0; p < 4; ++p) v[cc][p] = sc[p * step];
+                }
+            }
+#pragma unroll
+            for (int cc = 0; cc < CH; ++cc) {
+                if (c0 + cc >= C) break;
+                const bool neg = (c0 + cc == 0 && fy) || (c0 + cc == 1 && fx);
+#pragma unroll
+                for (int p = 0; p < 4; ++p) {
+                    const float x = neg ? -v[cc][p] : v[cc][p];
+                    acc[cc][p] = (float)((double)acc[cc][p] + (double)x * m[p]);
+                }
+            }
+        }
+    } else {
+        for (int p = 0; p < npx; ++p) {
+            for (int k = 0; k < K; ++k) {
+                const int2 e = tap_t[(size_t)k * HW + idx0 + p];
+                if (e.y < 0) break;
+                const bool fy = e.y & BT_FY, fx = e.y & BT_FX;
+                const double m = m_t[(size_t)k * HW + idx0 + p];
+                const float *s = src + (size_t)(e.y & 0xFFFF) * C * bb + e.x;
+#pragma unroll
+                for (int cc = 0; cc < CH; ++cc) {
+                    if (c0 + cc >= C) break;
+                    float x = s[(size_t)(c0 + cc) * bb];
+                    if ((c0 + cc == 0 && fy) || (c0 + cc == 1 && fx)) x = -x;
+#pragma unroll
+                    for (int pp = 0; pp < 4; ++pp)
+                        if (pp == p) acc[cc][pp] = (float)((double)acc[cc][pp] + (double)x * m);
+                }
+            }
+        }
+    }
+    double navg[4];
+#pragma unroll
+    for (int p = 0; p < 4; ++p) navg[p] = p < npx ? navg_t[idx0 + p] : 1.0;
+#pragma unroll
+    for (int cc = 0; cc < CH; ++cc) {
+        const int ch = c0 + cc;
+        if (ch >= C) break;
+        float *o = ch < 2 ? dP + (t * 2 + ch) * HW : ch == 2 ? cellprob + t * HW : logits + (t * ncls + (ch - 3)) * HW;
+        float r[4];
+#pragma unroll
+        for (int p = 0; p < 4; ++p) r[p] = (float)((double)acc[cc][p] / navg[p]);
+        if ((g.W & 3) == 0) {
+            *reinterpret_cast<float4 *>(o + idx0) = make_float4(r[0], r[1], r[2], r[3]);
+        } else {
+#pragma unroll
+            for (int p = 0; p < 4; ++p)
+                if (p < npx) o[idx0 + p] = r[p];
+        }
+    }
+}
+
+extern "C" size_t cpx_blend_table_bytes(const cpx_tiling *tiling) {
+    BlendTable L;
+    return blend_table_layout(tiling, &L) ? 0 : L.total;
+}
+
+extern "C" int cpx_blend_table_build(const cpx_tiling *tiling, const double *taper1d, void *table, size_t table_bytes,
+                                     void *stream) {
+    TilingDev g; int rc = tiling_to_dev(tiling, &g); if (rc) return rc;
+    BlendTable L; rc = blend_table_layout(tiling, &L); if (rc) return rc;
+    CPX_REQUIRE(taper1d && table && table_bytes >= L.total && ((uintptr_t)table & 255) == 0);
+    char *tb = (char *)table;
+    const int HW = g.H * g.W;
+    hipLaunchKernelGGL(k_blend_table, dim3(cpx_cdiv(HW, NTHR)), dim3(NTHR), 0, (hipStream_t)stream, g, taper1d, L.K,
+                       (double *)(tb + L.off_navg), (double *)(tb + L.off_m), (int2 *)(tb + L.off_tap));
+    if (g.W % 4 == 0)
+        hipLaunchKernelGGL(k_blend_table_hints, dim3(cpx_cdiv(HW / 4, NTHR)), dim3(NTHR), 0, (hipStream_t)stream, g, L.K,
+                           (int2 *)(tb + L.off_tap));
+    CPX_CHECK_LAUNCH();
+    return CPX_OK;
+}
+
+extern "C" int cpx_blend_planes(const float *planes, int ncls, int nT, const cpx_tiling *tiling, const void *table,
+                                size_t table_bytes, float *dP, float *cellprob, float *logits, void *stream) {
+    TilingDev g; int rc = tiling_to_dev(tiling, &g); if (rc) return rc;
+    BlendTable L; rc = blend_table_layout(tiling, &L); if (rc) return rc;
+    CPX_REQUIRE(planes && table && dP && cellprob && nT > 0 && ncls >= 0 && (ncls == 0 || logits));
+    CPX_REQUIRE(table_bytes >= L.total && ((uintptr_t)table & 255) == 0 && ((uintptr_t)planes & 15) == 0);
+    CPX_REQUIRE(g.W % 4 || (((uintptr_t)dP | (uintptr_t)cellprob | (uintptr_t)logits) & 15) == 0);
+    const char *tb = (const char *)table;
+    const int C = 3 + ncls, quads = g.H * ((g.W + 3) / 4);
+    const double *navg = (const double *)(tb + L.off_navg), *m = (const double *)(tb + L.off_m);
+    const int2 *tap = (const int2 *)(tb + L.off_tap);
+    constexpr int CH = 5;
+    if (C <= 3)
+        hipLaunchKernelGGL(k_blend_planes<3>, dim3(cpx_cdiv(quads, NTHR), nT, 1), dim3(NTHR), 0, (hipStream_t)stream, planes, C, ncls, g,
+                           L.K, navg, m, tap, dP, cellprob, logits);
+    else
+        hipLaunchKernelGGL(k_blend_planes<CH>, dim3(cpx_cdiv(quads, NTHR), nT, cpx_cdiv(C, CH)), dim3(NTHR), 0, (hipStream_t)stream, planes,
+                           C, ncls, g, L.K, navg, m, tap, dP, cellprob, logits);
+    CPX_CHECK_LAUNCH();
+    return CPX_OK;
+}
diff --git a/classpose_amd/engine.py b/classpose_amd/engine.py
--- a/classpose_amd/engine.py
+++ b/classpose_amd/engine.py
@@ -370,7 +370,7 @@
                  batch_tiles: int = 8, augment: bool = False, tile_overlap: float = 0.1,
                  niter: int = 200, cellprob_threshold: float = 0.0, flow_threshold: float = 0.4,
                  min_size: int = 15, max_size_fraction: float = 0.4, net_hw: tuple[int, int] | None = None,
-                 resample: bool = True):
+                 resample: bool = True, head_planes: bool = True):
         self.L = _lib.lib()
         self.w = weights
         self.dev = weights.device
@@ -397,6 +397,18 @@
                                                                 nT * self.n_sub, weights.c.dtype)
         self.net_ws = torch.empty(self.net_ws_bytes, dtype=torch.uint8, device=d)
         self.taper = torch.from_numpy(taper_1d(BSIZE)).to(d)
+        self.head_planes = bool(head_planes) and weights.c.dtype != _lib.DT_F32 and not weights.c.n_unet_ops
+        self.blend_table = None
+        if self.head_planes:
+            nb = self.L.cpx_blend_table_bytes(C.byref(self.tiling))
+            if not nb:
+                raise _lib.CpxError("cpx_blend_table_bytes: invalid tiling")
+            self.blend_table = torch.empty(nb, dtype=torch.uint8, device=d)
+            with torch.cuda.device(d):
+                st = torch.cuda.current_stream(d)
+                check(self.L.cpx_blend_table_build(C.byref(self.tiling), ptr(self.taper), ptr(self.blend_table), nb, st.cuda_stream),
+                      "blend_table_build")
+                st.synchronize()
         self.pp_ws_bytes = self.L.cpx_postproc_workspace_bytes(nT, H, W)
         self.max_rec = min(self.L.cpx_postproc_max_labels(H, W), 65535)
         self.max_pts = nT * max(4096, 2 * H * W)
@@ -450,8 +462,9 @@
                                       ptr(sl.patches), sn), "make_patches")
         if ev:
             ev[1].record(self.s_net)
-        check(self.L.cpx_net_forward(C.byref(self.w.c), ptr(sl.patches), self.nT * self.n_sub, ptr(sl.head),
-                                     ptr(self.net_ws), self.net_ws_bytes, sn), "net_forward")
+        net_forward = self.L.cpx_net_forward_planes if self.head_planes else self.L.cpx_net_forward
+        check(net_forward(C.byref(self.w.c), ptr(sl.patches), self.nT * self.n_sub, ptr(sl.head),
+                          ptr(self.net_ws), self.net_ws_bytes, sn), "net_forward")
         if ev:
             ev[2].record(self.s_net)
         sl.ev_net.record(self.s_net)
@@ -462,9 +475,14 @@
         ncls = self.w.ncls
         if ev:
             ev[3].record(self.s_post)
-        check(self.L.cpx_blend_subtiles(ptr(sl.head), self.w.c.ld_head, ncls if ncls > 1 else 0, n,
-                                        C.byref(self.tiling), ptr(self.taper), ptr(sl.dP),
-                                        ptr(sl.cellprob), ptr(sl.logits), sp), "blend")
+        if self.head_planes:
+            check(self.L.cpx_blend_planes(ptr(sl.head), ncls if ncls > 1 else 0, n, C.byref(self.tiling),
+                                          ptr(self.blend_table), self.blend_table.numel(), ptr(sl.dP),
+                                          ptr(sl.cellprob), ptr(sl.logits), sp), "blend")
+        else:
+            check(self.L.cpx_blend_subtiles(ptr(sl.head), self.w.c.ld_head, ncls if ncls > 1 else 0, n,
+                                            C.byref(self.tiling), ptr(self.taper), ptr(sl.dP),
+                                            ptr(sl.cellprob), ptr(sl.logits), sp), "blend")
         if ev:
             ev[4].record(self.s_post)
             tm.append(ev)
diff --git a/include/classpose_hip.h b/include/classpose_hip.h
--- a/include/classpose_hip.h
+++ b/include/classpose_hip.h
@@ -53,6 +53,12 @@
 int cpx_blend_subtiles_nchw(const float *y, const float *y_class, int ncls, int nT,
                             const cpx_tiling *tiling_host, const double *taper1d,
                             float *dP, float *cellprob, float *logits, void *stream);
+size_t cpx_blend_table_bytes(const cpx_tiling *tiling_host);
+int cpx_blend_table_build(const cpx_tiling *tiling_host, const double *taper1d, void *table,
+                          size_t table_bytes, void *stream);
+int cpx_blend_planes(const float *planes, int ncls, int nT, const cpx_tiling *tiling_host,
+                     const void *table, size_t table_bytes, float *dP, float *cellprob, float *logits,
+                     void *stream);
 
 typedef struct cpx_block_weights {
     const float *ln1_w, *ln1_b;
@@ -125,6 +131,8 @@
 int cpx_net_mlp_parts(int n_subtiles, int dtype);
 int cpx_net_forward(const cpx_net_weights *w_host, const void *patches, int n_subtiles,
                     float *head, void *workspace, size_t workspace_bytes, void *stream);
+int cpx_net_forward_planes(const cpx_net_weights *w_host, const void *patches, int n_subtiles,
+                           float *planes, void *workspace, size_t workspace_bytes, void *stream);
 
 #define CPX_PROF_N_KINDS 7
 int cpx_prof_create(int max_launches, int stride, unsigned kinds_mask, void **prof_out);
@@ -151,6 +159,7 @@
 #define CPX_EPI_POS_BF16 4
 #define CPX_EPI_RELU_BF16 5
 #define CPX_EPI_QKV_BF16 6
+#define CPX_EPI_F32_PLANES 7
 int cpx_gemm_bf16(const void *A, const void *Wt, int M, int N, int K, int epilogue,
                   const float *bias, const void *resid_or_pos, void *out, int ld_out,
                   void *stream);
```
